# mattpan-peregrinus/Cosmology_GNN_Simulation

Measured on AMD Instinct MI355X. Metric: particle-edge updates/sec (E x MP-steps), higher is better.
Workload: dtype bf16; 1 GPU; 1000000 particles/GPU (1000000 in all, weak scaling) uniform periodic box, k=16, latent=128, hidden=128, 10 MP rounds, edge MLP bf16 (f32 accumulate, f32 latents/LayerNorm/residual), node path fp16x2, message_source=x_j; particles_per_gpu=1000000, edges_per_gpu=16000000, k=16, latent=128, mp_steps=10, parallelism=single GPU

## Files before the change

cosmology_gnn_simulation_amd/_lib.py:

```python
from __future__ import annotations

import ctypes as C
import os
from typing import Optional

import torch

_HERE = os.path.dirname(os.path.abspath(__file__))
LIB_PATH = os.path.join(_HERE, "libcgnn_hip.so")

MAX_HIDDEN_LAYERS = 6
F32, BF16, BF16_N16, F32X3, F32X3_N16, F16X2_N16, F16X2 = 0, 1, 2, 3, 4, 5, 6
N16_NODE = (F32X3_N16, F16X2_N16)
P_F32, P_BF16_S32, P_BF16_S16, P_F16_S32 = 0, 1, 2, 3
STREAM_FOLDED = 1
LDS_WEIGHT_BUDGET = 152 * 1024
PRECISIONS = {"fp32": F32, "f32": F32, "float32": F32, "bf16": BF16, "bfloat16": BF16, "bf16_n16": BF16_N16,
              "fp32x3": F32X3, "f32x3": F32X3, "fp32x3_n16": F32X3_N16, "fp16x2_n16": F16X2_N16,
              "fp16x2": F16X2, "f16x2": F16X2}
F32_EMULATED = (F32X3, F16X2)

EXPORTS = (
    "cgnn_version", "cgnn_arch", "cgnn_last_error", "cgnn_packed_linear_bytes", "cgnn_pack_linear",
    "cgnn_mlp_rows", "cgnn_project_nodes", "cgnn_edge_block", "cgnn_aggregate", "cgnn_node_block",
    "cgnn_knn_workspace_bytes", "cgnn_knn_periodic", "cgnn_knn_sorted_order", "cgnn_segment_colsum",
    "cgnn_gather_rows", "cgnn_scatter_rows", "cgnn_tiled_rows", "cgnn_relayout", "cgnn_window_features",
    "cgnn_mlp_backward", "cgnn_weight_grad", "cgnn_weight_grad_x3_workspace_bytes", "cgnn_weight_grad_x3",
    "cgnn_col_dot", "cgnn_col_dot2", "cgnn_col_dot_workspace_bytes", "cgnn_col_dot_ordered", "cgnn_weight_grad_workspace_bytes", "cgnn_weight_grad_ordered", "cgnn_csr_workspace_bytes", "cgnn_csr_build",
    "cgnn_aggregate_csr", "cgnn_aggregate_csr_add", "cgnn_edge_stream", "cgnn_edge_stream_image_bytes", "cgnn_edge_stream_image_build",
    "cgnn_edge_stream_run", "cgnn_edge_stream_w8_supported", "cgnn_edge_stream_image_build_w8", "cgnn_edge_stream_run_w8", "cgnn_aggregate_plan_bytes", "cgnn_aggregate_plan_build", "cgnn_aggregate_planned", "cgnn_aggregate_planned_rows",
    "cgnn_aggregate_planned_form", "cgnn_edge_mlp_backward", "cgnn_linear2_rows", "cgnn_halo_return_add", "cgnn_window_features_rows",
    "cgnn_rollout_integrate", "cgnn_frame_unpack", "cgnn_training_sample",
    "cgnn_balanced_planes_workspace_bytes", "cgnn_balanced_planes", "cgnn_tile_classify",
    "cgnn_knn_adaptive_workspace_bytes", "cgnn_knn_periodic_adaptive", "cgnn_knn_adaptive_sorted_order",
    "cgnn_history_features", "cgnn_rollout_advance", "cgnn_halo_select", "cgnn_halo_pack", "cgnn_migrate_pack",
    "cgnn_migrate_unpack", "cgnn_knn_periodic_mode", "cgnn_knn_periodic_adaptive_mode",
    "cgnn_training_sample_backward", "cgnn_rollout_integrate_backward", "cgnn_edge_attr_backward",
    "cgnn_edge_attr_backward_rows", "cgnn_rows_to_frames", "cgnn_frame_grad_rows", "cgnn_mlp_rows_project",
    "cgnn_knn_batched_workspace_bytes", "cgnn_knn_periodic_batched", "cgnn_knn_batched_sorted_order",
    "cgnn_pair_counts_workspace_bytes", "cgnn_pair_counts", "cgnn_frame_errors_workspace_bytes", "cgnn_frame_errors",
    "cgnn_mass_assign", "cgnn_power_bin_ids", "cgnn_power_bins_workspace_bytes", "cgnn_power_bins",
    "cgnn_fof_labels_workspace_bytes", "cgnn_fof_labels", "cgnn_fof_catalogue", "cgnn_mass_assign_backward",
    "cgnn_mass_assign_weighted", "cgnn_mass_assign_weighted_backward",
    "cgnn_halo_match_workspace_bytes", "cgnn_halo_match", "cgnn_fof_group_sums",
    "cgnn_halo_profiles_workspace_bytes", "cgnn_halo_profiles",
    "cgnn_redshift_positions", "cgnn_power_multipoles_workspace_bytes", "cgnn_power_multipoles",
    "cgnn_pair_counts_smu_workspace_bytes", "cgnn_pair_counts_smu",
    "cgnn_pair_velocity_sums_workspace_bytes", "cgnn_pair_velocity_sums",
)
PAIR_COUNTS_MAX_BINS = 256
PAIR_COUNTS_SMU_MAX_BINS = 4096
PAIR_COUNTS_SMU_MAX_AXIS = 128
PAIR_VELOCITY_MAX_BINS = 64
MASS_ASSIGN_Q = 8192
MASS_ASSIGN_MAX_MESH = 512
MASS_ASSIGN_MAX_PARTICLES = 1 << 24
WEIGHT_BITS = 20
WEIGHTED_MAX_PARTICLES = 1 << 23
WEIGHTED_MAX_CHANNELS = 4
POWER_MAX_BINS = 256
POWER_MULTIPOLE_SUMS = 12
FOF_MAX_BINS = 256
FOF_DISP_UNITS = 1 << 30
HALO_MATCH_COLS = 6
GROUP_SUMS_MAX_CHANNELS = 4
HALO_PROFILES_MAX_BINS = 32
HALO_PROFILES_MAX_CHANNELS = 4
KNN_BATCH_GROUP = 64
KNN_EDGE_ATTR_REFERENCE, KNN_EDGE_ATTR_IMAGE = 0, 1
ROLLOUT_ROW = 5
MIGRATE_BLOCK = 256
MIGRATE_MAX_WORLD = 64
ROWS, TILED32 = 0, 1


class Linear(C.Structure):
    _fields_ = [("w", C.c_void_p), ("b", C.c_void_p), ("in_dim", C.c_int32), ("out_dim", C.c_int32)]


class Mlp(C.Structure):
    _fields_ = [("precision", C.c_int32), ("num_hidden_layers", C.c_int32),
                ("layer", Linear * (MAX_HIDDEN_LAYERS + 1)),
                ("ln_gamma", C.c_void_p), ("ln_beta", C.c_void_p)]


class MlpBwdBuffers(C.Structure):
    _fields_ = [("h", C.c_void_p * MAX_HIDDEN_LAYERS), ("g_a", C.c_void_p * MAX_HIDDEN_LAYERS),
                ("g_o", C.c_void_p), ("zhat", C.c_void_p)]


class CgnnError(RuntimeError):
    pass


_lib: Optional[C.CDLL] = None


def load() -> C.CDLL:
    global _lib
    if _lib is not None:
        return _lib
    if not os.path.isfile(LIB_PATH):
        raise CgnnError(
            f"{LIB_PATH} not found. Build the gfx950 kernels first: "
            "`python -c 'import __graft_entry__ as g; g.build()'` or "
            "`make -C cosmology_gnn_simulation_amd/csrc -j8`. There is no CPU fallback.")
    lib = C.CDLL(LIB_PATH)
    vp, i32, i64, sz, f32 = C.c_void_p, C.c_int32, C.c_int64, C.c_size_t, C.c_float
    lib.cgnn_version.restype = C.c_int
    lib.cgnn_arch.restype = C.c_char_p
    lib.cgnn_last_error.restype = C.c_char_p
    lib.cgnn_packed_linear_bytes.restype = sz
    lib.cgnn_packed_linear_bytes.argtypes = [i32, i32, i32]
    lib.cgnn_pack_linear.argtypes = [vp, i32, i32, i32, i32, i32, vp, vp]
    lib.cgnn_mlp_rows.argtypes = [C.POINTER(Mlp), vp, i64, i32, vp, i32, i32, vp]
    lib.cgnn_mlp_rows_project.argtypes = [C.POINTER(Mlp), vp, vp, i64, i32, vp, i32, C.POINTER(Linear), C.POINTER(Linear),
                                          i32, vp, vp, i32, vp]
    lib.cgnn_tiled_rows.restype = i64
    lib.cgnn_tiled_rows.argtypes = [i64]
    lib.cgnn_relayout.argtypes = [vp, i32, vp, i32, i64, i32, vp]
    lib.cgnn_project_nodes.argtypes = [C.POINTER(Linear), C.POINTER(Linear), i32, vp, i64, vp, vp, i32, vp]
    lib.cgnn_edge_block.argtypes = [C.POINTER(Mlp), vp, vp, vp, vp, i64, vp, vp, vp, i32, i32, vp, vp, i32, vp]
    lib.cgnn_edge_stream.argtypes = [C.POINTER(Mlp), i32, vp, vp, i64, vp, vp, i64, vp, vp, i32, C.POINTER(Mlp), vp, i32, vp]
    lib.cgnn_edge_stream_image_bytes.restype = sz
    lib.cgnn_edge_stream_image_bytes.argtypes = [i32, i32, i32, i32]
    lib.cgnn_edge_stream_image_build.argtypes = [C.POINTER(Mlp), i32, C.POINTER(Mlp), i32, vp, sz, vp]
    lib.cgnn_edge_stream_run.argtypes = [vp, sz, i32, i32, i32, i32, vp, vp, i64, vp, vp, i64, vp, vp, vp, i32, vp]
    lib.cgnn_edge_stream_w8_supported.argtypes = [i32, i32, i32]
    lib.cgnn_edge_stream_image_build_w8.argtypes = [C.POINTER(Mlp), i32, C.POINTER(Mlp), i32, vp, sz, vp]
    lib.cgnn_edge_stream_run_w8.argtypes = [vp, sz, i32, i32, i32, i32, vp, vp, i64, vp, vp, i64, vp, vp, vp, i32, i32, i32, i32, i32, vp]
    lib.cgnn_aggregate.argtypes = [vp, i32, vp, vp, i64, i32, i64, i32, vp, vp]
    lib.cgnn_aggregate_plan_bytes.restype = sz
    lib.cgnn_aggregate_plan_bytes.argtypes = [i64, i32]
    lib.cgnn_aggregate_plan_build.argtypes = [vp, i64, i32, vp, vp]
    lib.cgnn_aggregate_planned.argtypes = [vp, vp, vp, i64, i32, i32, vp, vp]
    lib.cgnn_aggregate_planned_rows.argtypes = [vp, i64, vp, vp, i64, i32, i32, vp, vp]
    lib.cgnn_aggregate_planned_form.restype = i32
    lib.cgnn_aggregate_planned_form.argtypes = [i64, i64, i32, i32]
    lib.cgnn_node_block.argtypes = [C.POINTER(Mlp), C.POINTER(Linear), C.POINTER(Linear), vp, vp, i64, vp, i32, i32,
                                    C.POINTER(Linear), C.POINTER(Linear), i32, vp, vp, i32, vp]
    lib.cgnn_knn_workspace_bytes.restype = sz
    lib.cgnn_knn_workspace_bytes.argtypes = [i64, i32]
    lib.cgnn_knn_periodic.argtypes = [vp, i64, f32, i32, vp, i64, vp, vp, vp, sz, vp]
    lib.cgnn_knn_sorted_order.argtypes = [vp, i64, vp, vp]
    lib.cgnn_knn_adaptive_workspace_bytes.restype = sz
    lib.cgnn_knn_adaptive_workspace_bytes.argtypes = [i64, i32]
    lib.cgnn_knn_periodic_adaptive.argtypes = [vp, i64, f32, i32, vp, i64, vp, vp, vp, sz, vp]
    lib.cgnn_knn_adaptive_sorted_order.argtypes = [vp, i64, vp, vp]
    lib.cgnn_knn_periodic_mode.argtypes = lib.cgnn_knn_periodic.argtypes + [i32]
    lib.cgnn_knn_periodic_adaptive_mode.argtypes = lib.cgnn_knn_periodic_adaptive.argtypes + [i32]
    lib.cgnn_knn_batched_workspace_bytes.restype = sz
    lib.cgnn_knn_batched_workspace_bytes.argtypes = [C.POINTER(i64), i32, i32]
    lib.cgnn_knn_periodic_batched.argtypes = [vp, C.POINTER(i64), i32, f32, i32, vp, vp, vp, sz, vp, i32]
    lib.cgnn_knn_batched_sorted_order.argtypes = [vp, C.POINTER(i64), i32, vp, vp]
    lib.cgnn_pair_counts_workspace_bytes.restype = sz
    lib.cgnn_pair_counts_workspace_bytes.argtypes = [i64, i64, i32]
    lib.cgnn_pair_counts.argtypes = [vp, i64, vp, i64, f32, C.POINTER(f32), i32, vp, vp, sz, vp]
    lib.cgnn_pair_counts_smu_workspace_bytes.restype = sz
    lib.cgnn_pair_counts_smu_workspace_bytes.argtypes = [i64, i64, i32, i32]
    lib.cgnn_pair_counts_smu.argtypes = [vp, i64, vp, i64, f32, C.POINTER(f32), i32, C.POINTER(f32), i32, i32, vp, vp, sz,
                                         vp]
    lib.cgnn_pair_velocity_sums_workspace_bytes.restype = sz
    lib.cgnn_pair_velocity_sums_workspace_bytes.argtypes = [i64, i64, i32]
    lib.cgnn_pair_velocity_sums.argtypes = [vp, vp, i64, vp, vp, i64, f32, C.POINTER(f32), i32, vp, vp, vp, sz,
                                            vp]
    lib.cgnn_frame_errors_workspace_bytes.restype = sz
    lib.cgnn_frame_errors_workspace_bytes.argtypes = [i64, i64]
    lib.cgnn_frame_errors.argtypes = [vp, vp, vp, vp, i64, i64, f32, vp, vp, sz, vp]
    lib.cgnn_mass_assign.argtypes = [vp, i64, i64, f32, i32, i32, vp, vp]
    lib.cgnn_mass_assign_backward.argtypes = [vp, vp, i64, i64, f32, i32, i32, C.c_double, vp, vp]
    lib.cgnn_mass_assign_weighted.argtypes = [vp, vp, i64, i64, i32, f32, i32, i32, vp, vp]
    lib.cgnn_mass_assign_weighted_backward.argtypes = [vp, vp, vp, i64, i64, i32, f32, i32, i32, C.c_double, C.c_double,
                                                       vp, vp, vp]
    lib.cgnn_fof_labels_workspace_bytes.restype = sz
    lib.cgnn_fof_labels_workspace_bytes.argtypes = [i64]
    lib.cgnn_fof_labels.argtypes = [vp, i64, f32, f32, vp, vp, sz, vp]
    lib.cgnn_fof_catalogue.argtypes = [vp, vp, i64, f32, vp, vp, C.POINTER(i32), i32, vp, vp]
    lib.cgnn_halo_match_workspace_bytes.restype = sz
    lib.cgnn_halo_match_workspace_bytes.argtypes = [i64]
    lib.cgnn_halo_match.argtypes = [vp, vp, vp, vp, i64, i32, i32, vp, vp, vp, vp, C.POINTER(i32), i32, vp, vp, sz,
                                    vp]
    lib.cgnn_fof_group_sums.argtypes = [vp, vp, i64, i32, vp, vp]
    lib.cgnn_halo_profiles_workspace_bytes.restype = sz
    lib.cgnn_halo_profiles_workspace_bytes.argtypes = [i64, i64]
    lib.cgnn_halo_profiles.argtypes = [vp, i64, vp, i64, f32, C.POINTER(f32), i32, vp, i32, vp, vp, vp, sz,
                                       vp]
    lib.cgnn_power_bin_ids.argtypes = [i32, C.POINTER(f32), i32, vp, vp]
    lib.cgnn_power_bins_workspace_bytes.restype = sz
    lib.cgnn_power_bins_workspace_bytes.argtypes = [i64, i32]
    lib.cgnn_power_bins.argtypes = [vp, vp, i64, i32, i32, vp, vp, i32, vp, vp, vp, sz, vp]
    lib.cgnn_redshift_positions.argtypes = [vp, vp, i64, i64, f32, i32, f32, vp, vp]
    lib.cgnn_power_multipoles_workspace_bytes.restype = sz
    lib.cgnn_power_multipoles_workspace_bytes.argtypes = [i64, i32]
    lib.cgnn_power_multipoles.argtypes = [vp, vp, vp, vp, i64, i32, i32, i32, vp, vp, i32, vp, vp, vp, sz, vp]
    lib.cgnn_segment_colsum.argtypes = [vp, vp, i64, i32, i32, vp, vp]
    lib.cgnn_window_features.argtypes = [vp, vp, vp, vp, i32, i64, f32, f32, f32, f32, f32, f32, vp, vp, vp]
    lib.cgnn_window_features_rows.argtypes = [vp, vp, i32, i64, vp, i64, f32, f32, f32, f32, f32, f32, vp, vp, vp]
    lib.cgnn_rollout_integrate.argtypes = [vp, vp, vp, i64, vp, vp, vp, i64, i64, vp, f32, f32, vp, vp]
    lib.cgnn_frame_unpack.argtypes = [vp, i64, i64, vp, vp, vp]
    lib.cgnn_training_sample.argtypes = [vp, vp, vp, vp, i32, i64, vp, i64, C.c_double, C.c_uint64, C.c_uint64, f32, f32,
                                         f32, f32, f32, f32, vp, vp, vp, vp, vp, vp, vp, vp]
    lib.cgnn_training_sample_backward.argtypes = [vp, vp, vp, vp, i32, i64, vp, i64, i32, f32, f32, f32, f32, vp, vp, vp,
                                                  vp]
    lib.cgnn_rollout_integrate_backward.argtypes = [vp, vp, i64, vp, f32, f32, vp, vp, vp, vp, vp, vp]
    lib.cgnn_edge_attr_backward.argtypes = [vp, vp, vp, i64, i32, vp, vp, vp, vp]
    lib.cgnn_edge_attr_backward_rows.argtypes = [vp, vp, vp, i64, i64, i32, vp, vp, vp, vp]
    lib.cgnn_rows_to_frames.argtypes = [vp, vp, vp, i32, i64, i64, vp, vp, vp]
    lib.cgnn_frame_grad_rows.argtypes = [vp, vp, i64, i64, vp, vp, vp]
    lib.cgnn_balanced_planes_workspace_bytes.restype = sz
    lib.cgnn_balanced_planes_workspace_bytes.argtypes = [i64, i32, i32, i32]
    lib.cgnn_balanced_planes.argtypes = [vp, i64, i32, i32, i32, vp, vp, vp, vp, vp, sz, vp]
    lib.cgnn_tile_classify.argtypes = [vp, i64, i32, i32, i32, vp, vp, vp, i32, C.POINTER(C.c_double),
                                       C.POINTER(C.c_double), C.c_double, C.c_double, vp, vp, vp, vp]
    dp = C.POINTER(C.c_double)
    lib.cgnn_history_features.argtypes = [vp, i32, i64, i64, i32, vp, i64, vp, f32, f32, f32, f32, f32, f32, vp, vp, vp]
    lib.cgnn_rollout_advance.argtypes = [vp, i32, i64, i64, i32, vp, vp, vp, vp, i64, vp, f32, f32, i32, i32, i32, i32, vp,
                                         vp, vp, vp, vp, vp, vp, vp]
    lib.cgnn_halo_select.argtypes = [vp, i64, i32, i32, dp, dp, C.c_double, C.c_double, vp, vp, vp, vp]
    lib.cgnn_halo_pack.argtypes = [vp, vp, i64, i32, vp, i64, vp, vp]
    lib.cgnn_migrate_pack.argtypes = [vp, i32, i64, i64, vp, vp, i32, i32, vp, vp, i64, vp, vp, i64, vp]
    lib.cgnn_migrate_unpack.argtypes = [vp, i64, i32, vp, i64, i64, vp, vp]
    lib.cgnn_gather_rows.argtypes = [vp, vp, i64, i32, vp, vp]
    lib.cgnn_scatter_rows.argtypes = [vp, vp, i64, i32, vp, vp]
    lib.cgnn_halo_return_add.argtypes = [vp, i64, vp, vp, vp, i64, i32, vp, i64, vp]
    lib.cgnn_mlp_backward.argtypes = [C.POINTER(Mlp), C.POINTER(Linear), C.POINTER(Mlp), C.POINTER(Linear), vp, i32, vp,
                                      i32, vp, i32, i64, C.POINTER(MlpBwdBuffers), vp, i32, vp, i32, vp]
    lib.cgnn_edge_mlp_backward.argtypes = [C.POINTER(Mlp), C.POINTER(Mlp), vp, vp, vp, vp, i64, vp, vp, vp,
                                           C.POINTER(MlpBwdBuffers), vp, vp, i32, vp]
    lib.cgnn_linear2_rows.argtypes = [C.POINTER(Linear), C.POINTER(Linear), i32, vp, vp, i64, vp, vp, vp, vp]
    lib.cgnn_weight_grad.argtypes = [vp, i32, i32, vp, i32, i32, i64, vp, i32, i32, vp, vp]
    lib.cgnn_csr_workspace_bytes.restype = sz
    lib.cgnn_csr_workspace_bytes.argtypes = [i64]
    lib.cgnn_csr_build.argtypes = [vp, vp, i64, i64, vp, vp, vp, sz, vp]
    lib.cgnn_aggregate_csr.argtypes = [vp, vp, vp, i64, i32, vp, vp]
    lib.cgnn_aggregate_csr_add.argtypes = [vp, vp, vp, i64, i32, vp, vp, vp, vp]
    lib.cgnn_weight_grad_x3_workspace_bytes.argtypes = []
    lib.cgnn_weight_grad_x3_workspace_bytes.restype = C.c_size_t
    lib.cgnn_weight_grad_x3.argtypes = [vp, i32, vp, i32, i64, vp, i32, i32, vp, vp, C.c_size_t, vp]
    lib.cgnn_col_dot.argtypes = [vp, i32, vp, i32, i64, i32, vp, vp]
    lib.cgnn_col_dot2.argtypes = [vp, i32, vp, i32, i64, i32, vp, vp, vp]
    lib.cgnn_col_dot_workspace_bytes.restype = sz
    lib.cgnn_weight_grad_workspace_bytes.restype = sz
    lib.cgnn_weight_grad_workspace_bytes.argtypes = [i64, i32, i32]
    lib.cgnn_weight_grad_ordered.argtypes = [vp, i32, i32, vp, i32, i32, i64, vp, i32, i32, vp, vp, sz, vp]
    lib.cgnn_col_dot_workspace_bytes.argtypes = [i64, i32]
    lib.cgnn_col_dot_ordered.argtypes = [vp, i32, vp, i32, i64, i32, vp, vp, vp, sz, vp]
    missing = [name for name in EXPORTS if not hasattr(lib, name)]
    if missing:
        raise CgnnError(f"{LIB_PATH} lacks {missing}: rebuild it (make -C cosmology_gnn_simulation_amd/csrc)")
    _lib = lib
    return lib


def check(rc: int, what: str) -> None:
    if rc != 0:
        msg = load().cgnn_last_error().decode("utf-8", "replace")
        raise CgnnError(f"{what} failed (status {rc}): {msg}")


def require_device(t: torch.Tensor, name: str) -> None:
    if not t.is_cuda:
        raise CgnnError(f"{name} must live on a HIP device (got {t.device}); this engine has no CPU path")


def stream_ptr(device: torch.device) -> int:
    return torch.cuda.current_stream(device).cuda_stream


def ptr(t: Optional[torch.Tensor]) -> Optional[int]:
    return None if t is None else t.data_ptr()


def f32c(t: torch.Tensor, name: str) -> torch.Tensor:
    require_device(t, name)
    if t.dtype != torch.float32:
        t = t.float()
    return t if t.is_contiguous() else t.contiguous()


def i32c(t: torch.Tensor, name: str) -> torch.Tensor:
    require_device(t, name)
    if t.dtype != torch.int32:
        t = t.to(torch.int32)
    return t if t.is_contiguous() else t.contiguous()
```

cosmology_gnn_simulation_amd/csrc/edge_stream32w.hip:

```cpp
#include <string.h>

#include <type_traits>

#include "s32.hpp"

namespace cgnn {

#define CGNN_W8_WAVES 8
#define CGNN_W8_BLOCK (CGNN_W8_WAVES * 64)
#define CGNN_W8_SLOTS 3
#define CGNN_IC(x) std::integral_constant<int, (x)> {}
#include "w8_dev.hpp"

template <int DT>
struct W8Geom {
    typedef S32Geom<DT> G;
    static constexpr int D = G::D, KS = G::KS;
    static constexpr unsigned STRIDE = G::STRIDE, VEC_OFF = G::VEC_OFF;
    static constexpr int PIECES = (int)(STRIDE / 1024u);
    static constexpr int NP = (PIECES + CGNN_W8_WAVES - 1) / CGNN_W8_WAVES;
    static constexpr unsigned LNBUF_OFF = CGNN_W8_SLOTS * STRIDE;
    static constexpr unsigned LNBUF_BYTES = 2u * D * 4u;
    static constexpr unsigned PDST_OFF = LNBUF_OFF + 2u * LNBUF_BYTES;
    static constexpr unsigned PDST_ROW = 256u + 16u;
    static constexpr unsigned PDST_BYTES = 4u * PDST_ROW;
    static constexpr unsigned PSST_OFF = PDST_OFF + CGNN_W8_WAVES * PDST_BYTES;
    static constexpr unsigned PSST_BYTES = 64u * (unsigned)D / 2u;
    static constexpr unsigned LDS = PSST_OFF + CGNN_W8_WAVES * PSST_BYTES;
    static_assert(LDS <= 160u * 1024u, "LDS budget");
};

template <class W, int LAG>
struct RingW {
    const char* image;
    int count;
    int wave, lane;
    int slot;
    int dma_chunk, dma_slot;
    CGNN_W8_STAMP_MEMBER
    __device__ __forceinline__ RingW(const char* img, int cnt, int w, int l)
        : image(img), count(cnt), wave(w), lane(l), slot(0), dma_chunk(0), dma_slot(0) {}
    __device__ __forceinline__ unsigned lds0() const { return (unsigned)(uintptr_t)(LdsWeightPtr)(cgnn_smem); }
    __device__ __forceinline__ unsigned base() const { return lds0() + (unsigned)slot * W::STRIDE; }
    __device__ __forceinline__ unsigned base_next() const {
        return lds0() + (unsigned)(slot + 1 == CGNN_W8_SLOTS ? 0 : slot + 1) * W::STRIDE;
    }
    __device__ __forceinline__ unsigned vec_addr() const { return base() + W::VEC_OFF; }
    __device__ __forceinline__ unsigned lnbuf(int which) const { return lds0() + W::LNBUF_OFF + (unsigned)which * W::LNBUF_BYTES; }
    __device__ __forceinline__ void piece(int i) {
        asm volatile("" ::: "memory");
#if defined(__HIP_DEVICE_COMPILE__)
        int idx = wave + CGNN_W8_WAVES * i;
        if (idx >= W::PIECES) idx -= CGNN_W8_WAVES;
        const unsigned off = (unsigned)idx * 1024u;
        char* dst = cgnn_smem + (unsigned)dma_slot * W::STRIDE + off;
        const __amdgpu_buffer_rsrc_t rsrc =
            __builtin_amdgcn_make_buffer_rsrc(const_cast<char*>(image), 0, (int)((unsigned)count * W::STRIDE), 0x00020000);
        __builtin_amdgcn_raw_ptr_buffer_load_lds(rsrc, (LdsVoidPtrG)dst, 16, (unsigned)lane * 16u,
                                                 (unsigned)dma_chunk * W::STRIDE + off, 0, 0);
#endif
        asm volatile("" ::: "memory");
    }
    __device__ __forceinline__ void dma_done() {
        dma_chunk = dma_chunk + 1 == count ? 0 : dma_chunk + 1;
        dma_slot = dma_slot + 1 == CGNN_W8_SLOTS ? 0 : dma_slot + 1;
    }
    __device__ __forceinline__ void prime() {
        for (int c = 0; c < CGNN_W8_SLOTS - 1 - LAG; ++c) {
            for (int i = 0; i < W::NP; ++i) piece(i);
            dma_done();
        }
        CGNN_S32_VMCNT(0);
        __builtin_amdgcn_s_barrier();
        asm volatile("" ::: "memory");
    }
    template <int EXTRA, int K0 = 17>
    __device__ __forceinline__ void interval_end() {
        CGNN_W8_STAMP(K0);
        if constexpr (w8dev::SLEEP > 0) __builtin_amdgcn_s_sleep(w8dev::SLEEP);
        vm_wait_const<(LAG ? 0 : (CGNN_W8_CARRY ? EXTRA : W::NP + EXTRA))>();
        asm volatile("s_waitcnt lgkmcnt(0)" ::: "memory");
        CGNN_W8_STAMP(K0 + 1);
        __builtin_amdgcn_s_barrier();
        asm volatile("" ::: "memory");
        CGNN_W8_STAMP(K0 + 2);
    }
    __device__ __forceinline__ void advance() { slot = slot + 1 == CGNN_W8_SLOTS ? 0 : slot + 1; }
    __device__ __forceinline__ void idle_interval() {
        for (int i = 0; i < W::NP; ++i) piece(i);
        dma_done();
        interval_end<0>();
    }
};

template <int N>
__device__ __forceinline__ void lds_wait2(u32x4& a, u32x4& b) {
    asm volatile("s_waitcnt lgkmcnt(%2)" : "+v"(a), "+v"(b) : "n"(N));
}

struct FragBuf {
    static constexpr int PD = CGNN_W8_PD, NBUF = PD + 1;
    u32x4 b[NBUF][CGNN_W8_GS];
};
template <int M>
struct WBlockGeom {
    static constexpr int GS = CGNN_W8_GS, NG = M / GS;
    static_assert(M % GS == 0 && (GS == 4 || GS == 2), "groups of four or two fragments");
    static constexpr int rot_after(int rot) { return (rot + NG) % FragBuf::NBUF; }
};
template <int M, int ROT>
__device__ __forceinline__ void wblock_request(FragBuf& fb, unsigned addr) {
    constexpr int GS = WBlockGeom<M>::GS, NG = WBlockGeom<M>::NG, PD = FragBuf::PD, NBUF = FragBuf::NBUF;
    const unsigned a = addr + (unsigned)(threadIdx.x & 63) * 16u;
    static_for_each([&](auto pc) __attribute__((always_inline)) {
        constexpr int p = decltype(pc)::value;
        if constexpr (p < NG) {
            static_for_each([&](auto jc) __attribute__((always_inline)) {
                constexpr int j = decltype(jc)::value;
                fb.b[(ROT + p) % NBUF][j] = lds_read_b128<(p * GS + j) * 1024>(a);
            }, std::make_integer_sequence<int, GS>{});
        }
    }, std::make_integer_sequence<int, PD>{});
}
template <int NROW, int KS, int ROT, bool CIN, bool COUT, class Fill>
__device__ __forceinline__ void wblockw(f32x16 (&acc)[NROW], const bf16x8 (&in)[KS], FragBuf& fb, unsigned addr, unsigned addr_next,
                                        const Fill& fill) {
    constexpr int M = NROW * KS, GS = WBlockGeom<M>::GS, NG = WBlockGeom<M>::NG, PD = FragBuf::PD, NBUF = FragBuf::NBUF;
    static_assert(!COUT || NG >= PD, "a block that requests the next one's fragments is at least PD groups long");
    const unsigned a = addr + (unsigned)(threadIdx.x & 63) * 16u;
    const unsigned an = addr_next + (unsigned)(threadIdx.x & 63) * 16u;
    (void)an;
    if constexpr (!CIN) wblock_request<M, ROT>(fb, addr);
    static_for_each([&](auto gc) __attribute__((always_inline)) {
        constexpr int g = decltype(gc)::value;
        constexpr int newer = COUT ? (PD - 1) * GS : ((g + PD - 1 < NG ? g + PD - 1 : NG - 1) - g) * GS;
        constexpr int bi = (ROT + g) % NBUF;
        if constexpr (GS == 4)
            lds_wait4<newer>(fb.b[bi][0], fb.b[bi][1], fb.b[bi][2], fb.b[bi][3]);
        else
            lds_wait2<newer>(fb.b[bi][0], fb.b[bi][1]);
        static_for_each([&](auto jc) __attribute__((always_inline)) {
            constexpr int j = decltype(jc)::value, m = g * GS + j, o = m / KS, ks = m % KS;
            acc[o] = __builtin_amdgcn_mfma_f32_32x32x16_bf16(__builtin_bit_cast(bf16x8, fb.b[bi][j]), in[ks], acc[o], 0, 0, 0);
            if constexpr (g + PD < NG)
                fb.b[(ROT + g + PD) % NBUF][j] = lds_read_b128<((g + PD) * GS + j) * 1024>(a);
            else if constexpr (COUT)
                fb.b[(ROT + g + PD) % NBUF][j] = lds_read_b128<((g + PD - NG) * GS + j) * 1024>(an);
            fill.template run<m>();
            __builtin_amdgcn_sched_barrier(0);
        }, std::make_integer_sequence<int, GS>{});
    }, std::make_integer_sequence<int, NG>{});
}

template <bool RELU, int DT, int T, int S>
__device__ __forceinline__ void packw_slice(bf16x8 (&out)[2 * DT], const f32x16 (&acc)[DT]) {
    u32x4 v;
    v[0] = pack_bf16(acc[T][8 * S + 0], acc[T][8 * S + 1]);
    v[1] = pack_bf16(acc[T][8 * S + 2], acc[T][8 * S + 3]);
    v[2] = pack_bf16(acc[T][8 * S + 4], acc[T][8 * S + 5]);
    v[3] = pack_bf16(acc[T][8 * S + 6], acc[T][8 * S + 7]);
    const bf16x8 b = __builtin_bit_cast(bf16x8, v);
    out[2 * T + S] = RELU ? relu_bf16(b) : b;
}

template <int DT, int T0, int T1>
__device__ __forceinline__ void bias_rowsw(f32x16 (&acc)[DT], unsigned vec_addr, int h) {
    if constexpr (w8dev::ABL_BIAS) return;
    const LdsVecPtr b = (LdsVecPtr)(uintptr_t)vec_addr;
#pragma unroll
    for (int t = T0; t < T1; ++t)
#pragma unroll
        for (int g = 0; g < 4; ++g) {
            const f32x4 v = *(LdsVec4Ptr)(b + 32 * t + 8 * g + 4 * h);
#pragma unroll
            for (int c = 0; c < 4; ++c) acc[t][4 * g + c] = v[c];
        }
}

struct LnStats {
    float rstd, nmr;
};
struct LnSums {
    float s[4], q[4];
};
__device__ __forceinline__ void ln_sums_clear(LnSums& a) {
#pragma unroll
    for (int i = 0; i < 4; ++i) a.s[i] = a.q[i] = 0.f;
}
template <bool ZM, int DT, int T, int S>
__device__ __forceinline__ void ln_sums_add(LnSums& a, const f32x16 (&acc)[DT]) {
#pragma unroll
    for (int i = 8 * S; i < 8 * S + 8; i += 4) {
#pragma unroll
        for (int c = 0; c < 4; ++c) {
            if constexpr (!ZM) a.s[c] += acc[T][i + c];
            a.q[c] = __builtin_fmaf(acc[T][i + c], acc[T][i + c], a.q[c]);
        }
    }
}
template <bool ZM, int DT>
__device__ __forceinline__ LnStats ln_stats_finish(const LnSums& a) {
    constexpr int D = 32 * DT;
    const float ex2 = half_swap_sum((a.q[0] + a.q[1]) + (a.q[2] + a.q[3])) * (1.0f / D);
    LnStats st;
    if constexpr (ZM) {
        st.rstd = __builtin_amdgcn_rsqf(ex2 + 1e-5f);
        st.nmr = 0.f;
    } else {
        const float mean = half_swap_sum((a.s[0] + a.s[1]) + (a.s[2] + a.s[3])) * (1.0f / D);
        st.rstd = __builtin_amdgcn_rsqf(__builtin_fmaxf(__builtin_fmaf(-mean, mean, ex2), 0.f) + 1e-5f);
        st.nmr = -mean * st.rstd;
    }
    return st;
}
template <bool RES, bool BETA, bool ZM, int DT, int K0, int K1>
__device__ __forceinline__ void ln_affine_w(const f32x16 (&acc)[DT], f32x16 (&ev)[DT], bf16x8 (&in)[2 * DT], unsigned lnv, int h,
                                            LnStats st) {
    if constexpr (K1 > K0) {
        constexpr int D = 32 * DT;
        const LdsVecPtr gp = (LdsVecPtr)(uintptr_t)lnv + 4 * h;
        f32x4 gm[2][2], bt[2][2];
#pragma unroll
        for (int gg = 0; gg < 2; ++gg) {
            gm[K0 & 1][gg] = *(LdsVec4Ptr)(gp + 32 * (K0 >> 1) + 8 * (2 * (K0 & 1) + gg));
            if constexpr (BETA) bt[K0 & 1][gg] = *(LdsVec4Ptr)(gp + D + 32 * (K0 >> 1) + 8 * (2 * (K0 & 1) + gg));
        }
        __builtin_amdgcn_sched_barrier(0);
        static_for_each([&](auto kc) __attribute__((always_inline)) {
            constexpr int k = decltype(kc)::value + K0, t = k >> 1, s = k & 1, cur = k & 1, nxt = cur ^ 1;
            if constexpr (k + 1 < K1) {
                constexpr int t1 = (k + 1) >> 1, s1 = (k + 1) & 1;
#pragma unroll
                for (int gg = 0; gg < 2; ++gg) {
                    gm[nxt][gg] = *(LdsVec4Ptr)(gp + 32 * t1 + 8 * (2 * s1 + gg));
                    if constexpr (BETA) bt[nxt][gg] = *(LdsVec4Ptr)(gp + D + 32 * t1 + 8 * (2 * s1 + gg));
                }
            }
            if constexpr (w8dev::ABL_LN) {
                packw_slice<false, DT, t, s>(in, acc);
#pragma unroll
                for (int i = 0; i < 8; ++i) ev[t][8 * s + i] += acc[t][8 * s + i];
            } else {
                float nrm[8], bs[8];
#pragma unroll
                for (int i = 0; i < 8; ++i) nrm[i] = ZM ? acc[t][8 * s + i] * st.rstd : __builtin_fmaf(acc[t][8 * s + i], st.rstd, st.nmr);
                __builtin_amdgcn_sched_barrier(0);
                if constexpr (BETA) {
#pragma unroll
                    for (int i = 0; i < 8; ++i) bs[i] = RES ? bt[cur][i >> 2][i & 3] + ev[t][8 * s + i] : bt[cur][i >> 2][i & 3];
                    __builtin_amdgcn_sched_barrier(0);
                } else {
                    static_assert(BETA || RES, "a pass without beta adds into the residual");
#pragma unroll
                    for (int i = 0; i < 8; ++i) bs[i] = ev[t][8 * s + i];
                }
#pragma unroll
                for (int i = 0; i < 8; ++i) ev[t][8 * s + i] = __builtin_fmaf(nrm[i], gm[cur][i >> 2][i & 3], bs[i]);
                __builtin_amdgcn_sched_barrier(0);
                u32x4 v;
#pragma unroll
                for (int x = 0; x < 4; ++x) v[x] = pack_bf16(ev[t][8 * s + 2 * x], ev[t][8 * s + 2 * x + 1]);
                in[2 * t + s] = __builtin_bit_cast(bf16x8, v);
            }
            __builtin_amdgcn_sched_barrier(0);
        }, std::make_integer_sequence<int, K1 - K0>{});
    }
}

template <int DT, int T0, int T1>
__device__ __forceinline__ void selp_rows(f32x16 (&acc)[DT], const bf16x8 (&ps)[2 * DT], const bf16x8 (&pd)[2 * DT], bf16x8 sel0,
                                          bf16x8 sel1) {
    if constexpr (w8dev::ABL_SEL) return;
    static_for_each([&](auto tc) __attribute__((always_inline)) {
        constexpr int t = decltype(tc)::value + T0;
        f32x16 c = {0.f, 0.f, 0.f, 0.f, 0.f, 0.f, 0.f, 0.f, 0.f, 0.f, 0.f, 0.f, 0.f, 0.f, 0.f, 0.f};
        c = __builtin_amdgcn_mfma_f32_32x32x16_bf16(sel0, ps[2 * t], c, 0, 0, 0);
        c = __builtin_amdgcn_mfma_f32_32x32x16_bf16(sel1, ps[2 * t + 1], c, 0, 0, 0);
        c = __builtin_amdgcn_mfma_f32_32x32x16_bf16(sel0, pd[2 * t], c, 0, 0, 0);
        c = __builtin_amdgcn_mfma_f32_32x32x16_bf16(sel1, pd[2 * t + 1], c, 0, 0, 0);
        acc[t] = c;
    }, std::make_integer_sequence<int, T1 - T0>{});
}

__device__ __forceinline__ float mix_add_lo(unsigned a, unsigned b) {
    float r;
    asm("v_fma_mix_f32 %0, %1, 1.0, %2 op_sel:[0,0,0] op_sel_hi:[1,0,1]" : "=v"(r) : "v"(a), "v"(b));
    return r;
}
__device__ __forceinline__ float mix_add_hi(unsigned a, unsigned b) {
    float r;
    asm("v_fma_mix_f32 %0, %1, 1.0, %2 op_sel:[1,0,1] op_sel_hi:[1,0,1]" : "=v"(r) : "v"(a), "v"(b));
    return r;
}
template <int DT, int T, int S>
__device__ __forceinline__ void addp_half(f32x16 (&acc)[DT], const bf16x8 (&ps)[2 * DT], const bf16x8 (&pd)[2 * DT]) {
    const u32x4 a = __builtin_bit_cast(u32x4, ps[2 * T + S]), b = __builtin_bit_cast(u32x4, pd[2 * T + S]);
#pragma unroll
    for (int x = 0; x < 4; ++x) {
        acc[T][8 * S + 2 * x] = mix_add_lo(a[x], b[x]);
        acc[T][8 * S + 2 * x + 1] = mix_add_hi(a[x], b[x]);
    }
}
template <int DT, int T0, int T1>
__device__ __forceinline__ void addp_rows(f32x16 (&acc)[DT], const bf16x8 (&ps)[2 * DT], const bf16x8 (&pd)[2 * DT]) {
    static_for_each([&](auto tc) __attribute__((always_inline)) {
        constexpr int t = decltype(tc)::value + T0;
#pragma unroll
        for (int s = 0; s < 2; ++s) {
            const u32x4 a = __builtin_bit_cast(u32x4, ps[2 * t + s]), b = __builtin_bit_cast(u32x4, pd[2 * t + s]);
#pragma unroll
            for (int x = 0; x < 4; ++x) {
                acc[t][8 * s + 2 * x] = mix_add_lo(a[x], b[x]);
                acc[t][8 * s + 2 * x + 1] = mix_add_hi(a[x], b[x]);
            }
        }
    }, std::make_integer_sequence<int, T1 - T0>{});
}

template <int DT, int NH, bool ENC, int LAG, bool PF16, bool FOLD>
__global__ __launch_bounds__(CGNN_W8_BLOCK, 2) void edge_stream32w_kernel(
    S32Args a, const __bf16* __restrict__ ps_all, const __bf16* __restrict__ pd_all, int64_t round_stride,
    const int32_t* __restrict__ src, const int32_t* __restrict__ dst, int64_t num_edges, const float* e_in, float* e_out,
    const float* __restrict__ attr, int ld_attr, int seg_k) {
    typedef W8Geom<DT> W;
    static_assert(DT == 4, "the sender-row staging is laid out for latent 128 (four lanes per 64-byte half line)");
    constexpr int D = W::D, KS = W::KS, NP = W::NP;
    const int lane = threadIdx.x & 63, r = lane & 31, h = lane >> 5;
    const int wave = __builtin_amdgcn_readfirstlane(threadIdx.x >> 6);
    const bool lagging = LAG != 0 && wave >= CGNN_W8_WAVES / 2;
    const int L = a.rounds;
    const int steps_per_tile = (ENC ? NH + 1 : 0) + L * (NH + 1);
    const int64_t tiles = (num_edges + 31) / 32;
    const TileRange tr = tile_range(tiles);
    const int64_t first0 = tr.first - wave;
    const int iters = __builtin_amdgcn_readfirstlane(
        first0 < tr.end ? (int)((tr.end - first0 + tr.stride - 1) / tr.stride) : 0);
    if (iters == 0) return;
    RingW<W, LAG> ring(a.image, steps_per_tile, wave, lane);
    CGNN_W8_STAMP_BEGIN(ring)
    ring.prime();
    if (lagging) ring.idle_interval();
    const bf16x8 sel0 = p32_selector(lane, 0), sel1 = p32_selector(lane, 1);

    f32x16 ev[DT], acc[DT];
    FragBuf fb;
    constexpr bool CARRY = CGNN_W8_CARRY && LAG == 0;
    auto rot_at = [](bool enc_first, int l) constexpr -> int {
        int r = 0;
        if (l >= 1) r = enc_first ? WBlockGeom<DT * 2>::rot_after(0) : WBlockGeom<DT * KS>::rot_after(0);
        for (int i = 1; i < l; ++i) r = WBlockGeom<DT * KS>::rot_after(r);
        return r;
    };
    (void)rot_at;
    bf16x8 inb[2][2 * DT];
    bf16x8 ps[2 * DT], pd[2 * DT];
    int lnpar = 0;
    LnStats lnst = {0.f, 0.f};
    constexpr int KA = CGNN_W8_LN_EARLY < 2 * DT ? CGNN_W8_LN_EARLY : 2 * DT;
    int64_t tile = tr.first < tr.end ? tr.first : tr.end - 1;
    bool valid = tr.first < tr.end;

    const unsigned pdst = ring.lds0() + W::PDST_OFF + (unsigned)wave * W::PDST_BYTES;
    const int kk = seg_k < 32 ? seg_k : 32;
    auto load_pd_chunk = [&](const __bf16* table, unsigned off) __attribute__((always_inline)) -> u32x4 {
#if defined(__HIP_DEVICE_COMPILE__)
        const __amdgpu_buffer_rsrc_t rsrc = __builtin_amdgcn_make_buffer_rsrc(const_cast<__bf16*>(table), 0, 0x7fffffff, 0x00020000);
        return __builtin_amdgcn_raw_buffer_load_b128(rsrc, (int)off, 0, 0);
#else
        return u32x4{0u, 0u, 0u, 0u};
#endif
    };
    auto park_pd = [&](u32x4 chunk) __attribute__((always_inline)) {
        *(__attribute__((address_space(3))) u32x4*)(uintptr_t)(pdst + (unsigned)(lane >> 4) * W::PDST_ROW + (unsigned)(lane & 15) * 16u) = chunk;
    };
    const unsigned pd_read = pdst + (unsigned)(r / kk) * W::PDST_ROW + (PF16 ? 4u : 8u) * (unsigned)h * 16u;
    auto pd_piece = [](int i) constexpr -> unsigned { return PF16 ? (unsigned)(((i >> 2) * 8 + (i & 3)) * 16) : (unsigned)(16 * i); };
    auto read_pd = [&]() __attribute__((always_inline)) {
#pragma unroll
        for (int i = 0; i < 2 * DT; ++i)
            pd[i] = __builtin_bit_cast(bf16x8, *(const __attribute__((address_space(3))) u32x4*)(uintptr_t)(pd_read + pd_piece(i)));
    };
    auto read_pd_row = [&](auto tc) __attribute__((always_inline)) {
        constexpr int t = decltype(tc)::value;
#pragma unroll
        for (int i = 2 * t; i < 2 * t + 2; ++i)
            pd[i] = __builtin_bit_cast(bf16x8, *(const __attribute__((address_space(3))) u32x4*)(uintptr_t)(pd_read + pd_piece(i)));
    };
    u32x4 pdchunk = {0u, 0u, 0u, 0u};

    const unsigned psst = ring.lds0() + W::PSST_OFF + (unsigned)wave * W::PSST_BYTES;
    const unsigned ps_cq = (unsigned)((lane & 3) ^ ((lane >> 4) & 3)) * 16u;
    const unsigned ps_read = psst + (unsigned)(r + 32 * h) * 64u + (unsigned)((r >> 2) & 3) * 16u;
    unsigned so_lo = 0, so_hi = 0;
    auto stage_ps = [&](auto sub_c, auto i_c, const __bf16* table) __attribute__((always_inline)) {
        constexpr int SUB = decltype(sub_c)::value, i = decltype(i_c)::value;
        (void)SUB, (void)i, (void)ps_cq;
        asm volatile("" ::: "memory");
#if defined(__HIP_DEVICE_COMPILE__)
        const __amdgpu_buffer_rsrc_t rsrc = __builtin_amdgcn_make_buffer_rsrc(const_cast<__bf16*>(table), 0, 0x7fffffff, 0x00020000);
        char* dstp = cgnn_smem + W::PSST_OFF + (unsigned)wave * W::PSST_BYTES + (unsigned)i * 1024u;
        __builtin_amdgcn_raw_ptr_buffer_load_lds(rsrc, (LdsVoidPtrG)dstp, 16, ((i & 1) ? so_hi : so_lo) + ps_cq,
                                                 PF16 ? (i >> 1) * 64 + SUB * 128 : (i >> 1) * D + SUB * 64, 0, 0);
#endif
        asm volatile("" ::: "memory");
    };
    auto read_ps = [&](auto sub_c) __attribute__((always_inline)) {
        constexpr int SUB = decltype(sub_c)::value;
#pragma unroll
        for (int c = 0; c < 4; ++c)
            ps[4 * SUB + c] = __builtin_bit_cast(
                bf16x8, *(const __attribute__((address_space(3))) u32x4*)(uintptr_t)(ps_read ^ ((unsigned)c << 4)));
    };
    auto pieces_at = [&](auto qc, auto mc) __attribute__((always_inline)) {
        constexpr int q = decltype(qc)::value, M = decltype(mc)::value;
        constexpr int P0 = CGNN_W8_PIECE_SLOT + NP <= M ? CGNN_W8_PIECE_SLOT : M - NP;
        if constexpr (q >= P0 && q < P0 + NP) ring.piece(q - P0);
    };

    struct TileIn {
        int src_lo, src_hi, dst_row;
        f32x4 q;
    };
    auto load_tile_in = [&](int64_t T, TileIn& ti) __attribute__((always_inline)) {
        const int64_t e = T * 32 + r;
        const int64_t ce = e < num_edges ? e : num_edges - 1;
        const int64_t e_lo = T * 32 + (lane >> 2), e_hi = e_lo + 16;
        ti.src_lo = src[e_lo < num_edges ? e_lo : num_edges - 1];
        ti.src_hi = src[e_hi < num_edges ? e_hi : num_edges - 1];
        const int groups = 32 / kk;
        const int j = (lane >> 4) < groups ? (lane >> 4) : groups - 1;
        const int64_t eg = T * 32 + (int64_t)j * kk;
        ti.dst_row = dst[eg < num_edges ? eg : num_edges - 1];
        if (ENC) ti.q = *reinterpret_cast<const f32x4*>(attr + ce * ld_attr);
    };
    TileIn nxt;
    load_tile_in(tile, nxt);

    for (int it = 0; it < iters; ++it) {
        const unsigned dchunk = (unsigned)nxt.dst_row * (unsigned)D * 2u + (unsigned)(lane & 15) * 16u;
        const int64_t tn = tile + tr.stride;
        const int64_t tile_next = tn < tr.end ? tn : tile;
        {
            so_lo = (unsigned)nxt.src_lo * (unsigned)D * 2u;
            so_hi = (unsigned)nxt.src_hi * (unsigned)D * 2u;
            const f32x4 q_now = nxt.q;
            load_tile_in(tile_next, nxt);
            if (ENC) {
                const int fin = a.enc_in_dim;
                float v[8];
#pragma unroll
                for (int jj = 0; jj < 8; ++jj) v[jj] = (jj < 4 && h == 0 && jj < fin) ? q_now[jj] : 0.f;
                u32x4 w;
                w[0] = pack_bf16(v[0], v[1]);
                w[1] = pack_bf16(v[2], v[3]);
                w[2] = pack_bf16(v[4], v[5]);
                w[3] = pack_bf16(v[6], v[7]);
                inb[0][0] = __builtin_bit_cast(bf16x8, w);
                const u32x4 z = {0u, 0u, 0u, 0u};
                inb[0][1] = __builtin_bit_cast(bf16x8, z);
            } else {
                load_tile<DT>(ev, e_in + tile * (32 * D), lane);
#pragma unroll
                for (int t = 0; t < DT; ++t)
#pragma unroll
                    for (int s = 0; s < 2; ++s) {
                        u32x4 w;
#pragma unroll
                        for (int x = 0; x < 4; ++x) w[x] = pack_bf16(ev[t][8 * s + 2 * x], ev[t][8 * s + 2 * x + 1]);
                        inb[0][2 * t + s] = __builtin_bit_cast(bf16x8, w);
                    }
                park_pd(load_pd_chunk(pd_all, dchunk));
                static_for_each([&](auto ic) __attribute__((always_inline)) { stage_ps(CGNN_IC(0), ic, ps_all); },
                                std::make_integer_sequence<int, 4>{});
                CGNN_S32_VMCNT(0);
                read_ps(CGNN_IC(0));
                asm volatile("s_waitcnt lgkmcnt(0)" ::: "memory");
                static_for_each([&](auto ic) __attribute__((always_inline)) { stage_ps(CGNN_IC(1), ic, ps_all); },
                                std::make_integer_sequence<int, 4>{});
                CGNN_S32_VMCNT(0);
                read_ps(CGNN_IC(1));
                read_pd();
            }
        }

        auto step_first = [&](auto enc_tag, auto pend_tag, int rr) __attribute__((always_inline)) {
            constexpr bool IS_ENC = decltype(enc_tag)::value;
            constexpr int PEND = decltype(pend_tag)::value;
            constexpr int KS0 = IS_ENC ? 2 : KS;
            constexpr bool INBLK = PF16 && CGNN_W8_PF16_INBLK && NH <= 2 && !IS_ENC && PEND != 0;
            CGNN_W8_STAMP(8);
            if constexpr (PEND != 0) {
                if constexpr (!IS_ENC) {
                    if constexpr (LAG == 0) CGNN_S32_VMCNT(0);
                    park_pd(pdchunk);
                    read_ps(CGNN_IC(0));
                    asm volatile("s_waitcnt lgkmcnt(0)" ::: "memory");
                    const __bf16* tps = ps_all + (int64_t)rr * round_stride;
                    static_for_each([&](auto ic) __attribute__((always_inline)) { stage_ps(CGNN_IC(1), ic, tps); },
                                    std::make_integer_sequence<int, 4>{});
                }
                ln_affine_w<PEND == 2, !(FOLD && PEND == 2), FOLD, DT, KA, 2 * DT>(acc, ev, inb[0], ring.lnbuf(lnpar ^ 1), h, lnst);
                if constexpr (!IS_ENC) {
                    if constexpr (INBLK) read_pd_row(CGNN_IC(0)); else read_pd();
                }
            }
            const unsigned base = ring.base();
            CGNN_W8_STAMP(9);
            constexpr bool REQ = CARRY && !IS_ENC && CGNN_W8_REQ_EARLY;
            if constexpr (REQ) wblock_request<DT * KS0, 0>(fb, base);
            if constexpr (IS_ENC) {
                bias_rowsw<DT, 0, DT>(acc, ring.vec_addr() + (unsigned)D * 4u, h);
            } else if constexpr (PEND != 0) {
                if constexpr (INBLK) {
                    addp_rows<DT, 0, 1>(acc, ps, pd);
                } else if constexpr (PF16) {
                    addp_rows<DT, 0, DT / 2>(acc, ps, pd);
                    CGNN_S32_VMCNT(0);
                    read_ps(CGNN_IC(1));
                    addp_rows<DT, DT / 2, DT>(acc, ps, pd);
                } else {
                    selp_rows<DT, 0, DT / 2>(acc, ps, pd, sel0, sel1);
                    CGNN_S32_VMCNT(0);
                    read_ps(CGNN_IC(1));
                    selp_rows<DT, DT / 2, DT>(acc, ps, pd, sel0, sel1);
                }
            } else {
                if constexpr (PF16) addp_rows<DT, 0, DT>(acc, ps, pd);
                else selp_rows<DT, 0, DT>(acc, ps, pd, sel0, sel1);
            }
            CGNN_W8_STAMP(10);
            const bf16x8 (&in0)[KS0] = reinterpret_cast<const bf16x8(&)[KS0]>(inb[0][0]);
            wblockw<DT, KS0, 0, REQ, CARRY>(acc, in0, fb, base, ring.base_next(), make_fill([&](auto qc) __attribute__((always_inline)) {
                constexpr int q = decltype(qc)::value, t = q / KS0 - 1, w = q % KS0;
                pieces_at(qc, CGNN_IC(DT * KS0));
                if constexpr (INBLK && t + 2 < DT) {
                    constexpr int tn = t + 2 < DT ? t + 2 : 0;
                    if constexpr (w == 0) {
                        if constexpr (tn == DT / 2) {
                            CGNN_S32_VMCNT(0);
                            read_ps(CGNN_IC(1));
                        }
                        read_pd_row(CGNN_IC(tn));
                    }
                    if constexpr (w == CGNN_W8_ADDP0) addp_half<DT, tn, 0>(acc, ps, pd);
                    if constexpr (w == CGNN_W8_ADDP1) addp_half<DT, tn, 1>(acc, ps, pd);
                }
                if constexpr (t >= 0 && w == (KS0 > 4 ? CGNN_W8_PK0 : (KS0 > 2 ? 1 : KS0 - 1))) packw_slice<true, DT, (t < 0 ? 0 : t), 0>(inb[1], acc);
                if constexpr (t >= 0 && w == (KS0 > 4 ? CGNN_W8_PK1 : KS0 - 1)) {
                    packw_slice<true, DT, (t < 0 ? 0 : t), 1>(inb[1], acc);
                    bias_rowsw<DT, (t < 0 ? 0 : t), (t < 0 ? 0 : t) + 1>(acc, ring.vec_addr(), h);
                }
            }));
            packw_slice<true, DT, DT - 1, 0>(inb[1], acc);
            packw_slice<true, DT, DT - 1, 1>(inb[1], acc);
            bias_rowsw<DT, DT - 1, DT>(acc, ring.vec_addr(), h);
            ring.dma_done();
            ring.template interval_end<0, 11>();
            ring.advance();
        };
        auto step_hidden = [&](auto enc_tag, auto lc) __attribute__((always_inline)) {
            constexpr int l = decltype(lc)::value;
            constexpr bool IS_ENC = decltype(enc_tag)::value;
            CGNN_W8_STAMP(14);
            wblockw<DT, KS, rot_at(IS_ENC, l), CARRY, CARRY>(acc, inb[l & 1], fb, ring.base(), ring.base_next(), make_fill([&](auto qc) __attribute__((always_inline)) {
                constexpr int q = decltype(qc)::value, t = q / KS - 1, w = q % KS;
                pieces_at(qc, CGNN_IC(DT * KS));
                if constexpr (t >= 0 && w == (KS > 4 ? CGNN_W8_PK0 : (KS > 2 ? 1 : KS - 1))) packw_slice<true, DT, (t < 0 ? 0 : t), 0>(inb[(l + 1) & 1], acc);
                if constexpr (t >= 0 && w == (KS > 4 ? CGNN_W8_PK1 : KS - 1)) {
                    packw_slice<true, DT, (t < 0 ? 0 : t), 1>(inb[(l + 1) & 1], acc);
                    bias_rowsw<DT, (t < 0 ? 0 : t), (t < 0 ? 0 : t) + 1>(acc, ring.vec_addr(), h);
                }
            }));
            packw_slice<true, DT, DT - 1, 0>(inb[(l + 1) & 1], acc);
            packw_slice<true, DT, DT - 1, 1>(inb[(l + 1) & 1], acc);
            bias_rowsw<DT, DT - 1, DT>(acc, ring.vec_addr(), h);
            ring.dma_done();
            ring.template interval_end<0, 15>();
            ring.advance();
        };
        auto step_last = [&](auto enc_tag, auto p_tag, auto res_tag, const __bf16* nps, const __bf16* npd) __attribute__((always_inline)) {
            constexpr bool WITH_P = decltype(p_tag)::value, RES = decltype(res_tag)::value, IS_ENC = decltype(enc_tag)::value;
            CGNN_W8_STAMP(0);
            CGNN_W8_STAMP(1);
            LnSums sums;
            ln_sums_clear(sums);
            wblockw<DT, KS, rot_at(IS_ENC, NH), CARRY, false>(acc, inb[NH & 1], fb, ring.base(), 0u, make_fill([&](auto qc) __attribute__((always_inline)) {
                constexpr int q = decltype(qc)::value, t = q / KS - 1, w = q % KS;
                pieces_at(qc, CGNN_IC(DT * KS));
                constexpr int PQ = CGNN_W8_PIECE_SLOT == 0 ? NP : 0;
                if constexpr (WITH_P && q >= PQ && q < PQ + 4) stage_ps(CGNN_IC(0), CGNN_IC(q - PQ), nps);
                if constexpr (WITH_P && q == PQ + 4) pdchunk = load_pd_chunk(npd, dchunk);
                if constexpr (t >= 0 && w == (KS > 4 ? CGNN_W8_SM0 : (KS > 2 ? 2 : KS - 1))) ln_sums_add<FOLD, DT, (t < 0 ? 0 : t), 0>(sums, acc);
                if constexpr (t >= 0 && w == (KS > 4 ? CGNN_W8_SM1 : KS - 1)) ln_sums_add<FOLD, DT, (t < 0 ? 0 : t), 1>(sums, acc);
            }));
            CGNN_W8_STAMP(2);
            ln_sums_add<FOLD, DT, DT - 1, 0>(sums, acc);
            ln_sums_add<FOLD, DT, DT - 1, 1>(sums, acc);
            lnst = ln_stats_finish<FOLD, DT>(sums);
            ln_affine_w<RES, !(FOLD && RES && WITH_P), FOLD, DT, 0, KA>(acc, ev, inb[0], ring.vec_addr() + (unsigned)D * 4u, h, lnst);
            if (wave < CGNN_W8_WAVES / 2) {
                const int idx = wave * 64 + lane;
                if (idx < 2 * D) {
                    const LdsVecPtr sp = (LdsVecPtr)(uintptr_t)(ring.vec_addr() + (unsigned)D * 4u);
                    const float v = sp[idx];
                    ((__attribute__((address_space(3))) float*)(uintptr_t)ring.lnbuf(lnpar))[idx] = v;
                }
            }
            lnpar ^= 1;
            ring.dma_done();
            ring.template interval_end<(WITH_P && (!CARRY || CGNN_W8_PIECE_SLOT == 0) ? 5 : 0), 3>();
            ring.advance();
        };
        auto hidden_steps = [&](auto enc_tag) __attribute__((always_inline)) {
            static_for_each([&](auto lc) __attribute__((always_inline)) {
                step_hidden(enc_tag, std::integral_constant<int, decltype(lc)::value + 1>{});
            }, std::make_integer_sequence<int, NH - 1>{});
        };
        constexpr std::true_type ENC_PASS{};
        constexpr std::false_type ROUND_PASS{};

        if (ENC) {
            step_first(ENC_PASS, CGNN_IC(0), 0);
            hidden_steps(ENC_PASS);
            step_last(ENC_PASS, std::true_type{}, std::false_type{}, ps_all, pd_all);
            step_first(ROUND_PASS, CGNN_IC(1), 0);
            hidden_steps(ROUND_PASS);
        } else {
            step_first(ROUND_PASS, CGNN_IC(0), 0);
            hidden_steps(ROUND_PASS);
        }
        for (int rr = 1; rr < L; ++rr) {
            step_last(ROUND_PASS, std::true_type{}, std::true_type{}, ps_all + (int64_t)rr * round_stride, pd_all + (int64_t)rr * round_stride);
            step_first(ROUND_PASS, CGNN_IC(2), rr);
            hidden_steps(ROUND_PASS);
        }
        step_last(ROUND_PASS, std::false_type{}, std::true_type{}, ps_all, pd_all);
        ln_affine_w<true, true, FOLD, DT, KA, 2 * DT>(acc, ev, inb[0], ring.lnbuf(lnpar ^ 1), h, lnst);

        if (valid) {
            float* const tb = e_out + tile * (32 * D);
#pragma unroll
            for (int t = 0; t < DT; ++t)
#pragma unroll
                for (int g = 0; g < 4; ++g) {
                    const f32x4 v = {ev[t][4 * g], ev[t][4 * g + 1], ev[t][4 * g + 2], ev[t][4 * g + 3]};
                    __builtin_nontemporal_store(v, reinterpret_cast<f32x4*>(tb + ((4 * t + g) * 64 + lane) * 4));
                }
        }
        if (tn < tr.end) {
            tile = tn;
        } else {
            valid = false;
        }
    }
    if (LAG != 0 && !lagging) ring.idle_interval();
    CGNN_W8_STAMP_END(wave, lane)
    CGNN_S32_VMCNT(0);
    __builtin_amdgcn_s_barrier();
}

template <int DT, int NH, int LAG, bool PF16, bool FOLD>
static int launch_w8(const S32Args& a, const __bf16* ps, const __bf16* pd, int64_t round_stride, const int32_t* src,
                     const int32_t* dst, int64_t num_edges, const float* e_in, float* e_out, const float* attr, int ld_attr,
                     int seg_k, hipStream_t st) {
    typedef W8Geom<DT> W;
    const bool enc = a.enc_in_dim > 0;
    auto kern = enc ? edge_stream32w_kernel<DT, NH, true, LAG, PF16, FOLD> : edge_stream32w_kernel<DT, NH, false, LAG, PF16, FOLD>;
    if (W::LDS > 48 * 1024) {
        int rc = ensure_dynamic_lds(reinterpret_cast<const void*>(kern), W::LDS, "hipFuncSetAttribute(edge_stream32w)");
        if (rc != CGNN_OK) return rc;
    }
    const int64_t tiles = (num_edges + 31) / 32;
    const int grid = grid_for_tiles(tiles, 1, CGNN_W8_WAVES);
    kern<<<grid, CGNN_W8_BLOCK, W::LDS, st>>>(a, ps, pd, round_stride, src, dst, num_edges, e_in, e_out, attr, ld_attr, seg_k);
    CGNN_W8_STAMP_REPORT(st, num_edges, grid, a.rounds + (enc ? 1 : 0), LAG)
    return check_hip(hipGetLastError(), "cgnn_edge_stream_run_w8 launch");
}

}

using namespace cgnn;

extern "C" int cgnn_edge_stream_image_build_w8(const cgnn_mlp* rounds, int32_t num_rounds, const cgnn_mlp* encoder,
                                               int32_t latent, void* image, size_t image_bytes, void* stream) {
    int rc = cgnn_edge_stream_image_build(rounds, num_rounds, encoder, latent, image, image_bytes, stream);
    if (rc != CGNN_OK) return rc;
    const size_t stride = s32_stride(latent);
    const int nh = rounds[0].num_hidden_layers;
    const int count = (num_rounds + (encoder ? 1 : 0)) * (nh + 1);
    hipStream_t st = (hipStream_t)stream;
    const size_t vbytes = (size_t)latent * 4, voff = (size_t)latent * latent * 2;
    char* img = (char*)image;
    rc = check_hip(hipMemcpyAsync(img + voff + vbytes, img + voff, vbytes, hipMemcpyDeviceToDevice, st), "hipMemcpyAsync(own bias)");
    for (int c = 0; c + 1 < count && rc == CGNN_OK; ++c)
        rc = check_hip(hipMemcpyAsync(img + (size_t)c * stride + voff, img + (size_t)(c + 1) * stride + voff, vbytes,
                                      hipMemcpyDeviceToDevice, st), "hipMemcpyAsync(bias, one chunk early)");
    if (rc == CGNN_OK) rc = check_hip(hipMemsetAsync(img + (size_t)(count - 1) * stride + voff, 0, vbytes, st), "hipMemsetAsync(last bias)");
    return rc;
}

extern "C" int cgnn_edge_stream_w8_supported(int32_t latent, int32_t num_hidden_layers, int32_t fixed_k) {
    const bool k_ok = fixed_k >= 8 && (fixed_k <= 32 ? 32 % fixed_k == 0 : fixed_k % 32 == 0);
    return (latent == 128 && num_hidden_layers >= 1 && num_hidden_layers <= 3 && k_ok) ? 1 : 0;
}

extern "C" int cgnn_edge_stream_run_w8(const void* image, size_t image_bytes, int32_t latent, int32_t num_hidden_layers,
                                       int32_t num_rounds, int32_t enc_in_dim, const void* ps_all, const void* pd_all,
                                       int64_t round_stride, const int32_t* src, const int32_t* dst, int64_t num_edges,
                                       const float* e_in, float* e_out, const float* edge_attr, int32_t ld_attr, int32_t lag,
                                       int32_t fixed_k, int32_t p_format, int32_t flags, void* stream) {
    if (!image || !ps_all || !pd_all || !src || !dst || !e_out || num_edges < 0 || num_rounds < 1 || num_hidden_layers < 1 ||
        round_stride < 0 || (enc_in_dim > 0 ? (!edge_attr || ld_attr < enc_in_dim) : !e_in) || lag < 0 || lag > 1 || fixed_k < 0) {
        set_error("cgnn_edge_stream_run_w8: invalid argument");
        return CGNN_ERR_INVALID_ARG;
    }
    if (p_format != CGNN_P_BF16_S32 && p_format != CGNN_P_F16_S32) {
        set_error("cgnn_edge_stream_run_w8: ps_all / pd_all must be CGNN_P_F16_S32 or CGNN_P_BF16_S32 tables (got p_format %d)",
                  p_format);
        return CGNN_ERR_INVALID_ARG;
    }
    if ((flags & ~CGNN_STREAM_FOLDED) != 0 || ((flags & CGNN_STREAM_FOLDED) && p_format != CGNN_P_F16_S32)) {
        set_error("cgnn_edge_stream_run_w8: flags = %d (known: CGNN_STREAM_FOLDED, with CGNN_P_F16_S32 tables only)", flags);
        return CGNN_ERR_INVALID_ARG;
    }
    if (p_format == CGNN_P_F16_S32 && lag != 0) {
        set_error("cgnn_edge_stream_run_w8: fp16 tables (CGNN_P_F16_S32) run with lag = 0 (lag = 1 is kept for bf16 tables)");
        return CGNN_ERR_UNSUPPORTED;
    }
    if (enc_in_dim > 4 || (enc_in_dim > 0 && ((ld_attr & 3) != 0 || ((uintptr_t)edge_attr & 15) != 0))) {
        set_error("cgnn_edge_stream_run_w8: the in-launch encoder reads an edge's features with one aligned 16-byte load: at most "
                  "4 features (got %d), ld_attr a multiple of 4 (got %d), edge_attr 16-byte aligned; other layouts: "
                  "cgnn_edge_stream_run", enc_in_dim, ld_attr);
        return CGNN_ERR_UNSUPPORTED;
    }
    if (!cgnn_edge_stream_w8_supported(latent, num_hidden_layers, fixed_k) || num_edges % fixed_k != 0) {
        set_error("cgnn_edge_stream_run_w8: no kernel for latent=%d, %d hidden layers, fixed_k=%d on %lld edges (built for latent "
                  "128, 1..3 hidden layers of the same width and receiver-sorted edge lists of fixed in-degree 8, 16, 32, 64, ...; "
                  "other shapes: cgnn_edge_stream_run)", latent, num_hidden_layers, fixed_k, (long long)num_edges);
        return CGNN_ERR_UNSUPPORTED;
    }
    const size_t need = cgnn_edge_stream_image_bytes(latent, num_hidden_layers, num_rounds, enc_in_dim > 0);
    if (image_bytes < need) {
        set_error("cgnn_edge_stream_run_w8: image has %zu bytes, this model needs %zu", image_bytes, need);
        return CGNN_ERR_INVALID_ARG;
    }
    if (num_edges == 0) return CGNN_OK;
    S32Args a;
    a.image = (const char*)image;
    a.rounds = num_rounds;
    a.nh = num_hidden_layers;
    a.enc_in_dim = enc_in_dim > 0 ? enc_in_dim : 0;
    hipStream_t st = (hipStream_t)stream;
#define CGNN_W8_GO(NHx, LAGx, PFx, FOLDx)                                                                                    \
    return launch_w8<4, NHx, LAGx, PFx, FOLDx>(a, (const __bf16*)ps_all, (const __bf16*)pd_all, round_stride, src, dst, num_edges, \
                                               e_in, e_out, edge_attr, ld_attr, fixed_k, st)
    if (flags & CGNN_STREAM_FOLDED) {
        switch (num_hidden_layers) {
            case 1: CGNN_W8_GO(1, 0, true, true);
            case 2: CGNN_W8_GO(2, 0, true, true);
            default: CGNN_W8_GO(3, 0, true, true);
        }
    }
    if (p_format == CGNN_P_F16_S32) {
        switch (num_hidden_layers) {
            case 1: CGNN_W8_GO(1, 0, true, false);
            case 2: CGNN_W8_GO(2, 0, true, false);
            default: CGNN_W8_GO(3, 0, true, false);
        }
    }
    if (lag) {
        switch (num_hidden_layers) {
            case 1: CGNN_W8_GO(1, 1, false, false);
            case 2: CGNN_W8_GO(2, 1, false, false);
            default: CGNN_W8_GO(3, 1, false, false);
        }
    }
    switch (num_hidden_layers) {
        case 1: CGNN_W8_GO(1, 0, false, false);
        case 2: CGNN_W8_GO(2, 0, false, false);
        default: CGNN_W8_GO(3, 0, false, false);
    }
#undef CGNN_W8_GO
}
```

cosmology_gnn_simulation_amd/csrc/w8_dev.hpp:

```cpp
#pragma once

#ifndef CGNN_W8_GS
#define CGNN_W8_GS 2
#endif
#ifndef CGNN_W8_PD
#define CGNN_W8_PD 2
#endif
#ifndef CGNN_W8_LN_EARLY
#define CGNN_W8_LN_EARLY 0
#endif
#ifndef CGNN_W8_PK0
#define CGNN_W8_PK0 2
#define CGNN_W8_PK1 4
#endif
#ifndef CGNN_W8_SM0
#define CGNN_W8_SM0 4
#define CGNN_W8_SM1 6
#endif
#ifndef CGNN_W8_PIECE_SLOT
#define CGNN_W8_PIECE_SLOT 16
#endif
#ifndef CGNN_W8_CARRY
#define CGNN_W8_CARRY 1
#endif
#ifndef CGNN_W8_REQ_EARLY
#define CGNN_W8_REQ_EARLY 1
#endif
#ifndef CGNN_W8_PF16_INBLK
#define CGNN_W8_PF16_INBLK 1
#endif
#ifndef CGNN_W8_ADDP0
#define CGNN_W8_ADDP0 5
#define CGNN_W8_ADDP1 6
#endif

namespace w8dev {
#ifdef CGNN_W8_ABL_LN
constexpr bool ABL_LN = true;
#else
constexpr bool ABL_LN = false;
#endif
#ifdef CGNN_W8_ABL_SEL
constexpr bool ABL_SEL = true;
#else
constexpr bool ABL_SEL = false;
#endif
#ifdef CGNN_W8_ABL_BIAS
constexpr bool ABL_BIAS = true;
#else
constexpr bool ABL_BIAS = false;
#endif
#ifdef CGNN_W8_SLEEP
constexpr int SLEEP = CGNN_W8_SLEEP;
#else
constexpr int SLEEP = 0;
#endif
}

#ifdef CGNN_W8_STAMPS
#include <stdio.h>
__device__ unsigned long long cgnn_w8_stamps[8 * 32];
struct W8Timer {
    unsigned long long sum[20], prev;
};
#define CGNN_W8_STAMP_MEMBER W8Timer tm;
#define CGNN_W8_STAMP(k)                                                                 \
    {                                                                                    \
        unsigned long long t_;                                                           \
        __builtin_amdgcn_sched_barrier(0);                                               \
        asm volatile("s_memtime %0\n\ts_waitcnt lgkmcnt(0)" : "=s"(t_)::"memory");       \
        __builtin_amdgcn_sched_barrier(0);                                               \
        tm.sum[k] += t_ - tm.prev;                                                       \
        tm.prev = t_;                                                                    \
    }
#define CGNN_W8_STAMP_BEGIN(ring)                                                            \
    auto& tm = ring.tm;                                                                      \
    for (int k = 0; k < 20; ++k) tm.sum[k] = 0;                                              \
    asm volatile("s_memtime %0\n\ts_waitcnt lgkmcnt(0)" : "=s"(tm.prev)::"memory");
#define CGNN_W8_STAMP_END(wave, lane)  \
    if (blockIdx.x == 8 && lane == 0)  \
        for (int k = 0; k < 20; ++k) cgnn_w8_stamps[wave * 32 + k] = tm.sum[k];
#define CGNN_W8_STAMP_REPORT(st, num_edges, grid, passes_per_tile, lag)                                                           \
    {                                                                                                                             \
        static int printed = 0;                                                                                                   \
        (void)hipStreamSynchronize(st);                                                                                           \
        if (printed++ == 2) {                                                                                                     \
            static unsigned long long hs[8 * 32];                                                                                 \
            (void)hipMemcpyFromSymbol(hs, HIP_SYMBOL(cgnn_w8_stamps), sizeof(hs));                                                \
            const char* names[20] = {"(gap)", "last: bias, P requests", "last: MFMAs", "last: LayerNorm part, copy",              \
                                     "last: vmcnt wait", "last: barrier", "", "", "(gap; tile ends)", "first: LayerNorm rest, Pd", \
                                     "first: P sums", "first: L0 + pack", "first: vmcnt wait", "first: barrier", "(gap)",          \
                                     "hidden: bias, MFMAs, pack", "hidden: vmcnt wait", "hidden: barrier / idle interval",         \
                                     "idle: vmcnt", "idle: barrier"};                                                              \
            const double passes = (double)(((num_edges) + 31) / 32) / ((grid) * 8.0) * (passes_per_tile);                          \
            printf("lag %d: cycles per pass and wave, by phase (sums over the wave's whole run / %.0f passes)\n", lag, passes);    \
            double tot[8] = {0};                                                                                                  \
            for (int k = 0; k < 20; ++k) {                                                                                        \
                bool any = false;                                                                                                 \
                for (int w = 0; w < 8; ++w) any |= hs[w * 32 + k] != 0;                                                           \
                if (!any) continue;                                                                                               \
                printf("  %2d %-28s", k, names[k]);                                                                               \
                for (int w = 0; w < 8; ++w) {                                                                                     \
                    printf(" %7.0f", hs[w * 32 + k] / passes);                                                                    \
                    tot[w] += hs[w * 32 + k] / passes;                                                                            \
                }                                                                                                                 \
                printf("\n");                                                                                                     \
            }                                                                                                                     \
            printf("     %-28s", "total");                                                                                        \
            for (int w = 0; w < 8; ++w) printf(" %7.0f", tot[w]);                                                                 \
            printf("\n");                                                                                                         \
        }                                                                                                                         \
    }
#else
#define CGNN_W8_STAMP_MEMBER
#define CGNN_W8_STAMP(k)
#define CGNN_W8_STAMP_BEGIN(ring)
#define CGNN_W8_STAMP_END(wave, lane)
#define CGNN_W8_STAMP_REPORT(st, num_edges, grid, passes_per_tile, lag)
#endif
```

cosmology_gnn_simulation_amd/ops.py:

```python
from __future__ import annotations

import ctypes as C
import math
import weakref
from typing import List, Optional, Sequence, Tuple

import torch

from . import _lib
from ._lib import BF16, BF16_N16, F32, CgnnError, Linear, Mlp, check, f32c, i32c, ptr, require_device, stream_ptr


_timer = None


class OpTimer:

    def __init__(self):
        self.records = {}

    def __enter__(self):
        global _timer
        _timer = self
        return self
# ... 58 lines not shown
        out_dim, ld = w.shape
        ncols = ld - col0 if ncols is None else ncols
        self.precision = _prec(precision)
        self.in_dim, self.out_dim = int(ncols), int(out_dim)
        nbytes = lib.cgnn_packed_linear_bytes(out_dim, ncols, self.precision)
        self.packed = torch.empty(nbytes, dtype=torch.uint8, device=w.device)
        with _timed("pack_linear", w.device):
            check(lib.cgnn_pack_linear(w.data_ptr(), out_dim, ld, col0, ncols, self.precision, self.packed.data_ptr(),
                                       stream_ptr(w.device)), "cgnn_pack_linear")
        self.bias = None if bias is None else f32c(bias.detach(), "bias").clone()

    def struct(self) -> Linear:
        return Linear(self.packed.data_ptr(), ptr(self.bias), self.in_dim, self.out_dim)


class PackedMLP:

    def __init__(self, linears: Sequence[Tuple[torch.Tensor, Optional[torch.Tensor]]],
                 layer_norm: Optional[Tuple[torch.Tensor, torch.Tensor]], precision,
                 first_layer_cols: Optional[Tuple[int, int]] = None):
        nh = len(linears) - 1
        if nh < 1 or nh > _lib.MAX_HIDDEN_LAYERS:
            raise CgnnError(f"mlp_num_hidden_layers={nh} outside [1, {_lib.MAX_HIDDEN_LAYERS}]")
        self.precision = _prec(precision)
        self.layers: List[PackedLinear] = []
        for i, (w, b) in enumerate(linears):
            if i == 0 and first_layer_cols is not None:
                self.layers.append(PackedLinear(w, b, self.precision, first_layer_cols[0], first_layer_cols[1]))
            else:
                self.layers.append(PackedLinear(w, b, self.precision))
        self.gamma = self.beta = None
        if layer_norm is not None:
            self.gamma = f32c(layer_norm[0].detach(), "ln weight").clone()
            self.beta = f32c(layer_norm[1].detach(), "ln bias").clone()
        self.num_hidden_layers = nh
        self.in_dim = self.layers[0].in_dim
        self.hidden = self.layers[0].out_dim
        self.out_dim = self.layers[-1].out_dim
        m = Mlp()
        m.precision = self.precision
        m.num_hidden_layers = nh
        for i, L in enumerate(self.layers):
            m.layer[i] = L.struct()
        m.ln_gamma = ptr(self.gamma)
        m.ln_beta = ptr(self.beta)
        self._struct = m

    def struct(self) -> Mlp:
        return self._struct

    def lds_bytes(self) -> int:
        pad16 = lambda n: (n * 4 + 15) // 16 * 16
        return sum(L.packed.numel() for L in self.layers) + sum(pad16(L.out_dim) for L in self.layers) + \
            2 * pad16(self.out_dim)


class TiledRows:

    def __init__(self, n: int, width: int, device, buf: Optional[torch.Tensor] = None):
        if width % 32:
            raise CgnnError(f"TILED32 needs a width that is a multiple of 32 (got {width})")
        self.n, self.width = int(n), int(width)
        rows = ((self.n + 31) // 32) * 32
        self.buf = buf if buf is not None else torch.empty((rows, width), dtype=torch.float32, device=device)
        if self.buf.shape != (rows, width) or not self.buf.is_contiguous():
            raise CgnnError("TiledRows: buffer has the wrong shape")

    @property
    def device(self):
        return self.buf.device

    def empty_like(self) -> "TiledRows":
        return TiledRows(self.n, self.width, self.buf.device)

    def to_rows(self) -> torch.Tensor:
        return relayout(self)

    @staticmethod
    def from_rows(x: torch.Tensor) -> "TiledRows":
        return relayout(x)


def relayout(x, out: Optional[torch.Tensor] = None):
    lib = _lib.load()
    if isinstance(x, TiledRows):
        if out is None:
            out = torch.empty((x.n, x.width), dtype=torch.float32, device=x.device)
        elif out.dtype != torch.float32 or not out.is_contiguous() or out.dim() != 2 or out.shape[1] != x.width or \
                out.shape[0] < x.n or out.device != x.device:
            raise CgnnError("relayout: out must be contiguous float32 [>= n, width] on the tiles' device")
        if x.n:
            with _timed("relayout", x.device):
                check(lib.cgnn_relayout(x.buf.data_ptr(), _lib.TILED32, out.data_ptr(), _lib.ROWS, x.n, x.width,
                                        stream_ptr(x.device)), "cgnn_relayout")
        return out
    x = f32c(x, "x")
    t = TiledRows(x.shape[0], x.shape[1], x.device)
    if t.n:
        with _timed("relayout", x.device):
            check(lib.cgnn_relayout(x.data_ptr(), _lib.ROWS, t.buf.data_ptr(), _lib.TILED32, t.n, t.width,
                                    stream_ptr(x.device)), "cgnn_relayout")
    return t


def mlp_rows(mlp: PackedMLP, x: torch.Tensor, out=None, tiled: bool = False, next_projection=None,
             index: Optional[torch.Tensor] = None):
    if not (mlp.precision == _lib.F16X2_N16 and torch.is_tensor(x) and x.is_cuda and x.dtype == torch.float32 and
            x.dim() == 2 and x.stride(1) == 1 and x.stride(0) >= x.shape[1]):
        x = f32c(x, "x")
    if x.dim() != 2 or x.shape[1] != mlp.in_dim:
        raise CgnnError(f"mlp_rows: input is {tuple(x.shape)}, the MLP expects [n, {mlp.in_dim}]")
    n = x.shape[0] if index is None else int(index.numel())
    if tiled or isinstance(out, TiledRows):
        y = out if out is not None else TiledRows(n, mlp.out_dim, x.device)
        yb, layout = y.buf, _lib.TILED32
    else:
        y = out if out is not None else torch.empty((n, mlp.out_dim), dtype=torch.float32, device=x.device)
        yb, layout = y, _lib.ROWS
    if next_projection is None and index is None:
        with _timed("mlp_rows", x.device):
            check(_lib.load().cgnn_mlp_rows(C.byref(mlp.struct()), x.data_ptr(), n, x.stride(0), yb.data_ptr(),
                                            yb.stride(0), layout, stream_ptr(x.device)), "cgnn_mlp_rows")
        return y
    if mlp.precision != _lib.F16X2_N16 or layout != _lib.ROWS:
        raise CgnnError("mlp_rows: next_projection / index need an 'fp16x2_n16' pack and row-major output")
    if index is not None:
        index = i32c(index, "index")
        if y.shape[0] < n or (mlp.gamma is None and x.shape[0] < n):
            raise CgnnError("mlp_rows: index is longer than the rows it addresses")
    if next_projection is not None:
        ws, wd, ps, pd, p_format = next_projection
        s1, s2 = ws.struct(), wd.struct()
        pdt = p_format_dtype(p_format)
        for t in (ps, pd):
            require_device(t, "projection table")
            if t.dtype != pdt or not t.is_contiguous() or t.shape != (n, ws.out_dim):
                raise CgnnError("mlp_rows: projection tables have the wrong dtype/shape")
        proj = (C.byref(s1), C.byref(s2), ws.precision, ps.data_ptr(), pd.data_ptr(), p_format)
    else:
        ps = pd = None
        proj = (None, None, 0, None, None, 0)
    _same_device(x, index, y, ps, pd)
    with _timed("mlp_rows", x.device):
        check(_lib.load().cgnn_mlp_rows_project(C.byref(mlp.struct()), x.data_ptr(), ptr(index), n, x.stride(0),
                                                yb.data_ptr(), yb.stride(0), *proj, stream_ptr(x.device)),
              "cgnn_mlp_rows_project")
    return y


def p_table_format(edge_mlp_precision) -> int:
    return {F32: _lib.P_F32, BF16: _lib.P_BF16_S32, BF16_N16: _lib.P_BF16_S16,
            _lib.F16X2_N16: _lib.P_F32, _lib.F16X2: _lib.P_F32}[_prec(edge_mlp_precision)]


def p_format_dtype(p_format: int) -> torch.dtype:
    return {_lib.P_F32: torch.float32, _lib.P_F16_S32: torch.float16}.get(p_format, torch.bfloat16)


def p_table_dtype(edge_mlp_precision) -> torch.dtype:
    return torch.float32 if _prec(edge_mlp_precision) in (F32, _lib.F16X2_N16, _lib.F16X2) else torch.bfloat16


def project_nodes(ws: Optional[PackedLinear], wd: Optional[PackedLinear], x: torch.Tensor,
                  ps: Optional[torch.Tensor] = None, pd: Optional[torch.Tensor] = None,
                  p_format: Optional[int] = None):
    x = f32c(x, "x")
    n = x.shape[0]
    ref = ws if ws is not None else wd
    if p_format is None:
        p_format = p_table_format(ref.precision)
    pdt = p_format_dtype(p_format)
    if ws is not None and ps is None:
        ps = torch.empty((n, ws.out_dim), dtype=pdt, device=x.device)
    if wd is not None and pd is None:
        pd = torch.empty((n, wd.out_dim), dtype=pdt, device=x.device)
    for t in (ps, pd):
        if t is not None and (t.dtype != pdt or not t.is_contiguous()):
            raise CgnnError(f"project_nodes: tables must be contiguous {pdt} for this precision")
    s1 = ws.struct() if ws is not None else None
    s2 = wd.struct() if wd is not None else None
    with _timed("project_nodes", x.device):
        check(_lib.load().cgnn_project_nodes(C.byref(s1) if s1 is not None else None,
                                         C.byref(s2) if s2 is not None else None, ref.precision, x.data_ptr(), n,
                                         ptr(ps) if ws is not None else None, ptr(pd) if wd is not None else None,
                                         p_format, stream_ptr(x.device)), "cgnn_project_nodes")
    return ps, pd


def edge_block(mlp: PackedMLP, ps: torch.Tensor, pd: torch.Tensor, src: torch.Tensor, dst: torch.Tensor,
               e_in: TiledRows, e_out: Optional[TiledRows] = None, e_upd: Optional[TiledRows] = None,
               residual: bool = True, agg_out: Optional[torch.Tensor] = None, x_gather: Optional[torch.Tensor] = None,
               seg_k: int = 0) -> TiledRows:
    if not isinstance(e_in, TiledRows):
        raise CgnnError("edge_block: edge latents must be TiledRows (use ops.relayout / TiledRows.from_rows)")
    src, dst = i32c(src, "src"), i32c(dst, "dst")
    ne, latent = e_in.n, e_in.width
    if e_out is None:
        e_out = e_in.empty_like()
    for t, name in ((ps, "ps"), (pd, "pd")):
        require_device(t, name)
        if not t.is_contiguous() or t.dtype != p_table_dtype(mlp.precision):
            raise CgnnError(f"edge_block: {name} must be a contiguous project_nodes table of the MLP's precision")
    for t in (e_out, e_upd):
        if t is not None and (t.n != ne or t.width != latent):
            raise CgnnError("edge_block: e_out / e_upd do not match the edge latents")
    if src.numel() != ne or dst.numel() != ne:
        raise CgnnError("edge_block: src/dst length does not match the edge latents")
    if agg_out is not None:
        if x_gather is not None:
            x_gather = f32c(x_gather, "x_gather")
            if x_gather.shape[1] != latent:
                raise CgnnError("edge_block: x_gather width must equal the latent size")
        if agg_out.dtype != torch.float32 or not agg_out.is_contiguous() or agg_out.shape[1] != latent:
            raise CgnnError("edge_block: agg_out must be contiguous float32 [receivers, latent]")
    _same_device(ps, pd, src, dst, e_in.buf, e_out.buf, x_gather, agg_out)
    with _timed("edge_block", e_in.device):
        check(_lib.load().cgnn_edge_block(C.byref(mlp.struct()), ps.data_ptr(), pd.data_ptr(), src.data_ptr(),
                                          dst.data_ptr(), ne, e_in.buf.data_ptr(), e_out.buf.data_ptr(),
                                          None if e_upd is None else e_upd.buf.data_ptr(),
                                          1 if residual else 0, latent, ptr(x_gather), ptr(agg_out), seg_k,
                                          stream_ptr(e_in.device)), "cgnn_edge_block")
    return e_out


def edge_stream(mlps: Sequence[PackedMLP], ps_all: torch.Tensor, pd_all: torch.Tensor, src: torch.Tensor,
                dst: torch.Tensor, e_in: Optional[TiledRows], e_out: Optional[TiledRows] = None,
                encoder: Optional[PackedMLP] = None, edge_attr: Optional[torch.Tensor] = None) -> TiledRows:
    src, dst = i32c(src, "src"), i32c(dst, "dst")
    rounds = len(mlps)
    ne = src.numel()
    if encoder is not None:
        if edge_attr is None:
            raise CgnnError("edge_stream: the encoder needs edge_attr")
        edge_attr = f32c(edge_attr, "edge_attr")
        if edge_attr.shape != (ne, encoder.in_dim) or encoder.precision != BF16_N16:
            raise CgnnError("edge_stream: edge_attr must be [E, encoder fan-in] and the encoder packed 'bf16_n16'")
        latent = encoder.out_dim
        if e_out is None:
            e_out = TiledRows(ne, latent, src.device)
    else:
        if not isinstance(e_in, TiledRows):
            raise CgnnError("edge_stream: edge latents must be TiledRows")
        latent = e_in.width
        if e_out is None:
            e_out = e_in.empty_like()
    for t, name in ((ps_all, "ps_all"), (pd_all, "pd_all")):
        require_device(t, name)
        if t.dtype != torch.bfloat16 or not t.is_contiguous() or t.dim() != 3 or t.shape[0] != rounds:
            raise CgnnError(f"edge_stream: {name} must be a contiguous bfloat16 [rounds, N, H] table")
    if any(m.precision != BF16_N16 for m in mlps):
        raise CgnnError("edge_stream: the edge models must be packed 'bf16_n16'")
    if dst.numel() != ne or e_out.n != ne or e_out.width != latent or (e_in is not None and e_in.n != ne):
        raise CgnnError("edge_stream: src/dst/e_out do not match the edge latents")
    arr = (Mlp * rounds)(*[m.struct() for m in mlps])
    enc = encoder.struct() if encoder is not None else None
    with _timed("edge_stream", src.device):
        check(_lib.load().cgnn_edge_stream(arr, rounds, ps_all.data_ptr(), pd_all.data_ptr(),
                                           ps_all.stride(0), src.data_ptr(), dst.data_ptr(), ne,
                                           e_in.buf.data_ptr() if e_in is not None else None, e_out.buf.data_ptr(), latent,
                                           C.byref(enc) if enc is not None else None, ptr(edge_attr),
                                           edge_attr.stride(0) if edge_attr is not None else 0,
                                           stream_ptr(src.device)), "cgnn_edge_stream")
    return e_out


class StreamImage:

    @staticmethod
    def supported(latent: int, hidden: int, nh: int, rounds: int, enc_in: Optional[int] = None) -> bool:
        if hidden != latent or rounds < 1 or (enc_in is not None and enc_in > 16):
            return False
        return _lib.load().cgnn_edge_stream_image_bytes(latent, nh, rounds, 1 if enc_in is not None else 0) > 0

    def __init__(self, mlps: Sequence[PackedMLP], encoder: Optional[PackedMLP] = None, kernel: str = "tile32",
                 folded: bool = False):
        lib = _lib.load()
        if kernel not in ("tile32", "tile32w"):
            raise CgnnError(f"StreamImage: unknown kernel {kernel!r}")
        self.kernel = kernel
        self.folded = bool(folded)
        self.rounds = len(mlps)
        self.latent = mlps[0].out_dim
        self.nh = mlps[0].num_hidden_layers
        self.enc_in = encoder.in_dim if encoder is not None else 0
        if any(m.precision != BF16 for m in mlps) or (encoder is not None and encoder.precision != BF16):
            raise CgnnError("StreamImage: the edge models must be packed 'bf16'")
        nbytes = lib.cgnn_edge_stream_image_bytes(self.latent, self.nh, self.rounds, 1 if encoder is not None else 0)
        if nbytes == 0:
            raise CgnnError(f"StreamImage: latent {self.latent} is not built (hidden == latent in {{32, 64, 128}})")
        dev = mlps[0].layers[0].packed.device
        self.buf = torch.empty(nbytes, dtype=torch.uint8, device=dev)
        arr = (Mlp * self.rounds)(*[m.struct() for m in mlps])
        enc = encoder.struct() if encoder is not None else None
        build = lib.cgnn_edge_stream_image_build_w8 if kernel == "tile32w" else lib.cgnn_edge_stream_image_build
        check(build(arr, self.rounds, C.byref(enc) if enc is not None else None, self.latent, self.buf.data_ptr(), nbytes,
                    stream_ptr(dev)), "cgnn_edge_stream_image_build")
        self._keep = (list(mlps), encoder)


def stream_w8_supported(latent: int, nh: int, fixed_k: int) -> bool:
    return bool(_lib.load().cgnn_edge_stream_w8_supported(latent, nh, int(fixed_k)))


def edge_stream_run(image: StreamImage, ps_all: torch.Tensor, pd_all: torch.Tensor, src: torch.Tensor, dst: torch.Tensor,
                    e_in: Optional[TiledRows], e_out: Optional[TiledRows] = None,
                    edge_attr: Optional[torch.Tensor] = None, kernel: str = "tile32", lag: int = 1,
                    fixed_k: int = 0, folded: Optional[bool] = None) -> TiledRows:
    if kernel not in ("tile32", "tile32w"):
        raise CgnnError(f"edge_stream_run: unknown kernel {kernel!r}")
    if image.kernel != kernel:
        raise CgnnError(f"edge_stream_run: the image was built for {image.kernel!r}, not {kernel!r} (StreamImage(..., kernel=...))")
    src, dst = i32c(src, "src"), i32c(dst, "dst")
    ne, latent = src.numel(), image.latent
    if image.enc_in:
        if edge_attr is None:
            raise CgnnError("edge_stream_run: this image starts with the encoder and needs edge_attr")
        edge_attr = f32c(edge_attr, "edge_attr")
        if edge_attr.shape != (ne, image.enc_in):
            raise CgnnError(f"edge_stream_run: edge_attr must be [E, {image.enc_in}]")
        e_in = None
    elif not isinstance(e_in, TiledRows) or e_in.n != ne or e_in.width != latent:
        raise CgnnError("edge_stream_run: e_in must be the TiledRows edge latents")
    if e_out is None:
        e_out = TiledRows(ne, latent, src.device) if e_in is None else e_in.empty_like()
    pdt = ps_all.dtype
    if pdt == torch.float16 and (kernel != "tile32w" or lag != 0):
        raise CgnnError("edge_stream_run: float16 (CGNN_P_F16_S32) tables are for kernel='tile32w' with lag=0")
    for t, name in ((ps_all, "ps_all"), (pd_all, "pd_all")):
        require_device(t, name)
        if t.dtype != pdt or pdt not in (torch.bfloat16, torch.float16) or not t.is_contiguous() or t.dim() != 3 or \
                t.shape[0] != image.rounds or t.shape[2] != latent:
            raise CgnnError(f"edge_stream_run: {name} must be a contiguous bfloat16 (or, tile32w, float16) "
                            f"[rounds, N, latent] table")
    if dst.numel() != ne or e_out.n != ne or e_out.width != latent:
        raise CgnnError("edge_stream_run: src/dst/e_out do not match the edge latents")
    args = (image.buf.data_ptr(), image.buf.numel(), latent, image.nh, image.rounds, image.enc_in, ps_all.data_ptr(),
            pd_all.data_ptr(), ps_all.stride(0), src.data_ptr(), dst.data_ptr(), ne,
            e_in.buf.data_ptr() if e_in is not None else None, e_out.buf.data_ptr(), ptr(edge_attr),
            edge_attr.stride(0) if edge_attr is not None else 0)
    with _timed("edge_stream", src.device):
        if kernel == "tile32w":
            fold = image.folded if folded is None else bool(folded)
            check(_lib.load().cgnn_edge_stream_run_w8(*args, int(lag), int(fixed_k),
                                                      _lib.P_F16_S32 if pdt == torch.float16 else _lib.P_BF16_S32,
                                                      _lib.STREAM_FOLDED if (fold and pdt == torch.float16) else 0,
                                                      stream_ptr(src.device)), "cgnn_edge_stream_run_w8")
        else:
            check(_lib.load().cgnn_edge_stream_run(*args, stream_ptr(src.device)), "cgnn_edge_stream_run")
    return e_out


class AggregatePlan:

    MIN_NODES = 8192

    def __init__(self, gather: torch.Tensor, num_nodes: int, fixed_k: int):
        gather = i32c(gather, "gather")
        if gather.numel() != num_nodes * fixed_k:
            raise CgnnError("AggregatePlan: gather must hold fixed_k senders per receiver")
        nbytes = _lib.load().cgnn_aggregate_plan_bytes(num_nodes, fixed_k)
        if nbytes == 0:
            raise CgnnError(f"AggregatePlan: fixed_k={fixed_k} cannot be planned")
        self._gather_ref = weakref.ref(gather)
        self.gather_ptr, self.device = gather.data_ptr(), gather.device
        self.num_nodes, self.fixed_k = num_nodes, fixed_k
        self.version = gather._version
        self.blob = torch.empty(nbytes, dtype=torch.uint8, device=gather.device)
        with _timed("aggregate_plan", gather.device):
            check(_lib.load().cgnn_aggregate_plan_build(gather.data_ptr(), num_nodes, fixed_k, self.blob.data_ptr(),
                                                        stream_ptr(gather.device)), "cgnn_aggregate_plan_build")

    @staticmethod
    def supported(num_nodes: int, fixed_k: int, width: int) -> bool:
        return 0 < fixed_k <= 32 and width % 32 == 0 and num_nodes >= AggregatePlan.MIN_NODES

    @staticmethod
    def of(gather: torch.Tensor, num_nodes: int, fixed_k: int, width: int) -> Optional["AggregatePlan"]:
        if not AggregatePlan.supported(num_nodes, fixed_k, width) or gather.dtype != torch.int32 or not gather.is_cuda:
            return None
        plan = getattr(gather, "_cgnn_aggregate_plan", None)
        if plan is None or plan.version != gather._version or plan.num_nodes != num_nodes or plan.fixed_k != fixed_k:
            plan = AggregatePlan(gather, num_nodes, fixed_k)
            gather._cgnn_aggregate_plan = plan
        return plan


def power_bin_ids(mesh: int, k_edges, device) -> torch.Tensor:
    what = "power_bin_ids"
    e = check_power_edges(k_edges, what)
    m = check_mesh(mesh, what)
    device = torch.device(device)
    if device.type != "cuda":
        raise CgnnError(f"{what}: needs a HIP device (got {device}); this engine has no CPU path")
    ids = torch.empty((m, m, m // 2 + 1), dtype=torch.int32, device=device)
    edges_c = (C.c_float * len(e))(*e)
    with _timed(what, ids.device):
        check(_lib.load().cgnn_power_bin_ids(m, edges_c, len(e) - 1, ids.data_ptr(), stream_ptr(ids.device)),
              "cgnn_power_bin_ids")
    return ids


class PowerPlan:

    _last = {}

    def __init__(self, mesh: int, k_edges, device):
        self.edges = tuple(check_power_edges(k_edges, "PowerPlan"))
        self.mesh, self.num_bins = check_mesh(mesh, "PowerPlan"), len(self.edges) - 1
        ids = power_bin_ids(self.mesh, self.edges, device).reshape(-1)
        self.device, self.num_modes = ids.device, ids.numel()
        sorted_ids, perm = torch.sort(ids, stable=True)
        del ids
        self.perm = perm.to(torch.int32)
        del perm
        self.bin_start = torch.searchsorted(
            sorted_ids, torch.arange(self.num_bins + 1, dtype=torch.int32, device=self.device)).to(torch.int32)

    @staticmethod
    def forget() -> None:
        PowerPlan._last.clear()

    @staticmethod
    def of(mesh: int, k_edges, device) -> "PowerPlan":
        device = torch.device(device)
        if device.type == "cuda" and device.index is None:
            device = torch.device("cuda", torch.cuda.current_device())
        key = (int(mesh), tuple(check_power_edges(k_edges, "PowerPlan")))
        plan = PowerPlan._last.get(device)
        if plan is None or (plan.mesh, plan.edges) != key:
            plan = PowerPlan(mesh, k_edges, device)
            PowerPlan._last[device] = plan
        return plan


def aggregate(table, gather: Optional[torch.Tensor], dst: Optional[torch.Tensor], num_nodes: int,
              fixed_k: int = 0, num_edges: Optional[int] = None, out: Optional[torch.Tensor] = None,
              plan: Optional[AggregatePlan] = None) -> torch.Tensor:
    if plan is not None:
        table = f32c(table, "table")
        if gather is None or gather.data_ptr() != plan.gather_ptr or gather.dtype != torch.int32:
            raise CgnnError("aggregate: the plan was built for another sender list")
        if plan.version != gather._version:
            raise CgnnError("aggregate: the sender list changed after the plan was built")
        if fixed_k != plan.fixed_k or num_nodes != plan.num_nodes or table.shape[1] % 32:
            raise CgnnError("aggregate: the plan does not match this call")
        if out is None:
            out = torch.empty((num_nodes, table.shape[1]), dtype=torch.float32, device=table.device)
        _same_device(table, gather, plan.blob, out)
        with _timed("aggregate", table.device):
            check(_lib.load().cgnn_aggregate_planned_rows(table.data_ptr(), table.shape[0], gather.data_ptr(),
                                                          plan.blob.data_ptr(), num_nodes, fixed_k, table.shape[1],
                                                          out.data_ptr(), stream_ptr(table.device)),
                  "cgnn_aggregate_planned")
        return out
    if isinstance(table, TiledRows):
        tb, layout, width, dev, nrows = table.buf, _lib.TILED32, table.width, table.device, table.n
    else:
        table = f32c(table, "table")
        tb, layout, width, dev, nrows = table, _lib.ROWS, table.shape[1], table.device, table.shape[0]
    if gather is not None:
        gather = i32c(gather, "gather")
    if dst is not None:
        dst = i32c(dst, "dst")
    if num_edges is None:
        num_edges = gather.numel() if gather is not None else (dst.numel() if dst is not None else nrows)
    if gather is None and nrows < num_edges:
        raise CgnnError(f"aggregate: a table of {nrows} rows read by edge id for {num_edges} edges")
    if out is None:
        out = torch.empty((num_nodes, width), dtype=torch.float32, device=dev)
    elif tuple(out.shape) != (num_nodes, width) or out.dtype != torch.float32 or not out.is_contiguous():
        raise CgnnError(f"aggregate: out must be contiguous float32 {(num_nodes, width)}")
    _same_device(tb, gather, dst, out)
    with _timed("aggregate", dev):
        check(_lib.load().cgnn_aggregate(tb.data_ptr(), layout, ptr(gather), ptr(dst), num_edges, fixed_k, num_nodes,
                                         width, out.data_ptr(), stream_ptr(dev)), "cgnn_aggregate")
    return out


def node_block(mlp: PackedMLP, w_x: PackedLinear, w_agg: PackedLinear, x: torch.Tensor, agg: torch.Tensor,
               x_out: Optional[torch.Tensor] = None, residual: bool = True, next_projection=None) -> torch.Tensor:
    x, agg = f32c(x, "x"), f32c(agg, "agg")
    n, latent = x.shape
    if x_out is None:
        x_out = torch.empty_like(x)
    sx, sa = w_x.struct(), w_agg.struct()
    if next_projection is not None:
        ws, wd, ps, pd, p_format = next_projection
        s1, s2 = ws.struct(), wd.struct()
        pdt = p_format_dtype(p_format)
        for t in (ps, pd):
            require_device(t, "projection table")
            if t.dtype != pdt or not t.is_contiguous() or t.shape != (n, ws.out_dim):
                raise CgnnError("node_block: projection tables have the wrong dtype/shape")
        proj = (C.byref(s1), C.byref(s2), ws.precision, ps.data_ptr(), pd.data_ptr(), p_format)
    else:
        proj = (None, None, 0, None, None, 0)
    _same_device(x, agg, x_out)
    with _timed("node_block", x.device):
        check(_lib.load().cgnn_node_block(C.byref(mlp.struct()), C.byref(sx), C.byref(sa), x.data_ptr(), agg.data_ptr(),
                                          n, x_out.data_ptr(), 1 if residual else 0, latent, *proj,
                                          stream_ptr(x.device)), "cgnn_node_block")
    return x_out


KNN_GRIDS = ("uniform", "adaptive")


def check_knn_grid(grid: str, who: str) -> str:
    if grid not in KNN_GRIDS:
        raise ValueError(f"{who}: k-NN grid {grid!r}; known: {KNN_GRIDS}")
    return grid


def check_min_image(flag: bool, who: str) -> bool:
    if not isinstance(flag, bool):
        raise TypeError(f"{who}: min_image_edge_attr must be a bool, got {flag!r}")
    return flag


def knn_periodic(pos: torch.Tensor, box_size: float, k: int, query_ids: Optional[torch.Tensor] = None,
                 want_edge_attr: bool = True, want_order: bool = False, *, min_image_edge_attr: bool = False,
                 grid: str = "uniform"):
    check_knn_grid(grid, "knn_periodic")
    check_min_image(min_image_edge_attr, "knn_periodic")
    lib = _lib.load()
    if grid == "adaptive":
        ws_fn, knn_fn, order_fn = (lib.cgnn_knn_adaptive_workspace_bytes, lib.cgnn_knn_periodic_adaptive,
                                   lib.cgnn_knn_adaptive_sorted_order)
        if min_image_edge_attr:
            knn_fn = lib.cgnn_knn_periodic_adaptive_mode
    else:
        ws_fn, knn_fn, order_fn = lib.cgnn_knn_workspace_bytes, lib.cgnn_knn_periodic, lib.cgnn_knn_sorted_order
        if min_image_edge_attr:
            knn_fn = lib.cgnn_knn_periodic_mode
    mode = (_lib.KNN_EDGE_ATTR_IMAGE,) if min_image_edge_attr else ()
    pos = f32c(pos, "pos")
    if pos.dim() != 2 or pos.shape[1] != 3:
        raise CgnnError(f"knn_periodic: pos must be [n, 3], got {tuple(pos.shape)}")
    n = pos.shape[0]
    if query_ids is not None:
        query_ids = i32c(query_ids, "query_ids")
        nq = query_ids.numel()
    else:
        nq = n
    ws_bytes = ws_fn(n, k)
    ws = torch.empty(ws_bytes, dtype=torch.uint8, device=pos.device)
    senders = torch.empty(nq * k, dtype=torch.int32, device=pos.device)
    edge_attr = torch.empty((nq * k, 4), dtype=torch.float32, device=pos.device) if want_edge_attr else None
    st = stream_ptr(pos.device)
    with _timed("knn_periodic", pos.device):
        check(knn_fn(pos.data_ptr(), n, float(box_size), k, ptr(query_ids), nq, senders.data_ptr(),
                     ptr(edge_attr), ws.data_ptr(), ws_bytes, st, *mode), knn_fn.__name__)
    order = None
    if want_order:
        order = torch.empty(n, dtype=torch.int32, device=pos.device)
        check(order_fn(ws.data_ptr(), n, order.data_ptr(), st), order_fn.__name__)
    return senders, edge_attr, order


def check_batch_offsets(offsets, who: str) -> List[int]:
    if torch.is_tensor(offsets):
        if offsets.is_cuda:
            raise CgnnError(f"{who}: offsets are host values (a list or a CPU tensor), got a tensor on {offsets.device}")
        offsets = offsets.tolist()
    offsets = [int(o) for o in offsets]
    if len(offsets) < 2 or offsets[0] != 0 or any(b <= a for a, b in zip(offsets, offsets[1:])):
        raise ValueError(f"{who}: offsets must hold B + 1 >= 2 strictly increasing values starting at 0, got {offsets}")
    return offsets


def knn_periodic_batched(pos: torch.Tensor, offsets, box_size: float, k: int, want_edge_attr: bool = True,
                         want_order: bool = False, *, min_image_edge_attr: bool = False, grid: str = "uniform"):
    what = "knn_periodic_batched"
    check_knn_grid(grid, what)
    check_min_image(min_image_edge_attr, what)
    offsets = check_batch_offsets(offsets, what)
    pos = f32c(pos, "pos")
    if pos.dim() != 2 or pos.shape[1] != 3 or pos.shape[0] != offsets[-1]:
        raise CgnnError(f"{what}: pos must be [{offsets[-1]}, 3] (offsets[-1] rows), got {tuple(pos.shape)}")
    n, num_graphs, k = offsets[-1], len(offsets) - 1, int(k)
    if grid == "adaptive":
        parts = [knn_periodic(pos[a:b], box_size, k, None, want_edge_attr, want_order,
                              min_image_edge_attr=min_image_edge_attr, grid="adaptive")
                 for a, b in zip(offsets, offsets[1:])]
        return (torch.cat([p[0] + a for p, a in zip(parts, offsets)]),
                torch.cat([p[1] for p in parts]) if want_edge_attr else None,
                torch.cat([p[2] + a for p, a in zip(parts, offsets)]) if want_order else None)
    lib = _lib.load()
    offs = (C.c_int64 * (num_graphs + 1))(*offsets)
    ws_bytes = lib.cgnn_knn_batched_workspace_bytes(offs, num_graphs, k)
    ws = torch.empty(ws_bytes, dtype=torch.uint8, device=pos.device)
    senders = torch.empty(n * k, dtype=torch.int32, device=pos.device)
    edge_attr = torch.empty((n * k, 4), dtype=torch.float32, device=pos.device) if want_edge_attr else None
    mode = _lib.KNN_EDGE_ATTR_IMAGE if min_image_edge_attr else _lib.KNN_EDGE_ATTR_REFERENCE
    st = stream_ptr(pos.device)
    with _timed(what, pos.device):
        check(lib.cgnn_knn_periodic_batched(pos.data_ptr(), offs, num_graphs, float(box_size), k, senders.data_ptr(),
                                            ptr(edge_attr), ws.data_ptr(), ws_bytes, st, mode),
              "cgnn_knn_periodic_batched")
    order = None
    if want_order:
        order = torch.empty(n, dtype=torch.int32, device=pos.device)
        check(lib.cgnn_knn_batched_sorted_order(ws.data_ptr(), offs, num_graphs, order.data_ptr(), st),
              "cgnn_knn_batched_sorted_order")
    return senders, edge_attr, order


def check_pair_count_edges(edges, box_size: float, who: str) -> List[float]:
    box = torch.tensor(float(box_size), dtype=torch.float32)
    if not (bool(torch.isfinite(box)) and float(box) > 0.0):
        raise ValueError(f"{who}: box_size must be positive and finite, got {box_size!r}")
    e = torch.as_tensor(edges).detach().to(device="cpu", dtype=torch.float32).reshape(-1)
    nb = e.numel() - 1
    if not 1 <= nb <= _lib.PAIR_COUNTS_MAX_BINS:
        raise ValueError(f"{who}: edges must hold nb + 1 radii with 1 <= nb <= {_lib.PAIR_COUNTS_MAX_BINS}, got "
                         f"{e.numel()} values")
    if not bool(torch.isfinite(e).all()) or float(e[0]) < 0.0 or not bool((e[1:] > e[:-1]).all()):
        raise ValueError(f"{who}: edges must be finite, start at 0 or above and ascend strictly (in float32)")
    if not bool(e[-1] <= box * 0.5):
        raise ValueError(f"{who}: the largest radius {float(e[-1])} exceeds half the box, {float(box) * 0.5}")
    return e.tolist()


def _check_in_box(what: str, box_size: float, **positions) -> None:
    for name, p in positions.items():
        if p is not None and not bool(((p >= 0) & (p <= float(box_size))).all()):
            raise ValueError(f"{what}: {name} leaves [0, box_size]")


def _pair_frames(what: str, pos_a, pos_b, box_size: float, check_bounds: bool):
    pos_a = f32c(pos_a, "pos_a")
    batched = pos_a.dim() == 3
    if pos_a.dim() not in (2, 3) or pos_a.shape[-1] != 3 or pos_a.shape[-2] < 1:
        raise CgnnError(f"{what}: pos_a must be [N, 3] or [T, N, 3] with N >= 1, got {tuple(pos_a.shape)}")
    if pos_b is not None:
        pos_b = f32c(pos_b, "pos_b")
        if pos_b.dim() != pos_a.dim() or pos_b.shape[-1] != 3 or pos_b.shape[-2] < 1 or \
                (batched and pos_b.shape[0] != pos_a.shape[0]):
            raise CgnnError(f"{what}: pos_b must be [M, 3] (or [T, M, 3] with pos_a's T) with M >= 1, got "
                            f"{tuple(pos_b.shape)} for pos_a {tuple(pos_a.shape)}")
        _same_device(pos_a, pos_b)
    if check_bounds:
        _check_in_box(what, box_size, pos_a=pos_a, pos_b=pos_b)
    if batched:
        return pos_a, pos_b, True
    return pos_a.unsqueeze(0), None if pos_b is None else pos_b.unsqueeze(0), False


# ... 1690 lines not shown
```

include/cgnn.h:

```cpp
#ifndef CGNN_H_
#define CGNN_H_

#include <stddef.h>
#include <stdint.h>

#ifdef __cplusplus
extern "C" {
#endif

#define CGNN_VERSION 100
#define CGNN_MAX_HIDDEN_LAYERS 6

typedef enum {
    CGNN_OK = 0,
    CGNN_ERR_INVALID_ARG = -1,
    CGNN_ERR_UNSUPPORTED = -2,
    CGNN_ERR_WORKSPACE = -3,
    CGNN_ERR_HIP = -4
} cgnn_status;

typedef enum {
    CGNN_F32 = 0,
    CGNN_BF16 = 1,
    CGNN_BF16_N16 = 2,
    CGNN_F32X3 = 3,
    CGNN_F32X3_N16 = 4,
    CGNN_F16X2_N16 = 5,
    CGNN_F16X2 = 6
} cgnn_precision;

typedef enum { CGNN_P_F32 = 0, CGNN_P_BF16_S32 = 1, CGNN_P_BF16_S16 = 2, CGNN_P_F16_S32 = 3 } cgnn_ptable;

typedef enum { CGNN_ROWS = 0, CGNN_TILED32 = 1 } cgnn_layout;

typedef struct {
    const void* w;
    const float* b;
    int32_t in_dim;
    int32_t out_dim;
} cgnn_linear;

typedef struct {
    int32_t precision;
    int32_t num_hidden_layers;
    cgnn_linear layer[CGNN_MAX_HIDDEN_LAYERS + 1];
    const float* ln_gamma;
    const float* ln_beta;
} cgnn_mlp;

int cgnn_version(void);
const char* cgnn_arch(void);
const char* cgnn_last_error(void);

size_t cgnn_packed_linear_bytes(int32_t out_dim, int32_t ncols, int32_t precision);
int cgnn_pack_linear(const float* w, int32_t out_dim, int32_t ld, int32_t col0, int32_t ncols,
                     int32_t precision, void* packed, void* stream);

int cgnn_mlp_rows(const cgnn_mlp* mlp, const float* x, int64_t n, int32_t ld_x,
                  float* y, int32_t ld_y, int32_t y_layout, void* stream);

int cgnn_mlp_rows_project(const cgnn_mlp* mlp, const float* x, const int32_t* index, int64_t n, int32_t ld_x, float* y,
                          int32_t ld_y, const cgnn_linear* ws, const cgnn_linear* wd, int32_t proj_precision, void* ps,
                          void* pd, int32_t p_format, void* stream);

int64_t cgnn_tiled_rows(int64_t n);
int cgnn_relayout(const float* src, int32_t from, float* dst, int32_t to, int64_t n, int32_t width, void* stream);

int cgnn_project_nodes(const cgnn_linear* ws, const cgnn_linear* wd, int32_t precision,
                       const float* x, int64_t n, void* ps, void* pd, int32_t p_format, void* stream);

int cgnn_edge_block(const cgnn_mlp* mlp, const void* ps, const void* pd,
                    const int32_t* src, const int32_t* dst, int64_t num_edges,
                    const float* e_in, float* e_out, float* e_upd, int32_t residual,
                    int32_t latent, const float* x_gather, float* agg_out, int32_t seg_k, void* stream);

int cgnn_aggregate(const float* table, int32_t table_layout, const int32_t* gather, const int32_t* dst,
                   int64_t num_edges, int32_t fixed_k, int64_t num_nodes, int32_t width,
                   float* out, void* stream);

size_t cgnn_aggregate_plan_bytes(int64_t num_nodes, int32_t fixed_k);
int cgnn_aggregate_plan_build(const int32_t* gather, int64_t num_nodes, int32_t fixed_k, void* plan, void* stream);
int cgnn_aggregate_planned(const float* table, const int32_t* gather, const void* plan, int64_t num_nodes,
                           int32_t fixed_k, int32_t width, float* out, void* stream);
int cgnn_aggregate_planned_rows(const float* table, int64_t table_rows, const int32_t* gather, const void* plan,
                                int64_t num_nodes, int32_t fixed_k, int32_t width, float* out, void* stream);
int32_t cgnn_aggregate_planned_form(int64_t table_rows, int64_t num_nodes, int32_t fixed_k, int32_t width);

int cgnn_node_block(const cgnn_mlp* mlp, const cgnn_linear* w_x, const cgnn_linear* w_agg,
                    const float* x, const float* agg, int64_t n, float* x_out,
                    int32_t residual, int32_t latent,
                    const cgnn_linear* ws_next, const cgnn_linear* wd_next, int32_t proj_precision,
                    void* ps_next, void* pd_next, int32_t p_format, void* stream);

int cgnn_edge_stream(const cgnn_mlp* rounds, int32_t num_rounds, const void* ps_all, const void* pd_all,
                     int64_t round_stride, const int32_t* src, const int32_t* dst, int64_t num_edges,
                     const float* e_in, float* e_out, int32_t latent, const cgnn_mlp* encoder, const float* edge_attr,
                     int32_t ld_attr, void* stream);

size_t cgnn_edge_stream_image_bytes(int32_t latent, int32_t num_hidden_layers, int32_t num_rounds, int32_t with_encoder);
int cgnn_edge_stream_image_build(const cgnn_mlp* rounds, int32_t num_rounds, const cgnn_mlp* encoder, int32_t latent,
                                 void* image, size_t image_bytes, void* stream);
int cgnn_edge_stream_run(const void* image, size_t image_bytes, int32_t latent, int32_t num_hidden_layers,
                         int32_t num_rounds, int32_t enc_in_dim, const void* ps_all, const void* pd_all,
                         int64_t round_stride, const int32_t* src, const int32_t* dst, int64_t num_edges,
                         const float* e_in, float* e_out, const float* edge_attr, int32_t ld_attr, void* stream);

#define CGNN_STREAM_FOLDED 1
int cgnn_edge_stream_w8_supported(int32_t latent, int32_t num_hidden_layers, int32_t fixed_k);
int cgnn_edge_stream_image_build_w8(const cgnn_mlp* rounds, int32_t num_rounds, const cgnn_mlp* encoder, int32_t latent,
                                    void* image, size_t image_bytes, void* stream);
int cgnn_edge_stream_run_w8(const void* image, size_t image_bytes, int32_t latent, int32_t num_hidden_layers,
                            int32_t num_rounds, int32_t enc_in_dim, const void* ps_all, const void* pd_all,
                            int64_t round_stride, const int32_t* src, const int32_t* dst, int64_t num_edges,
                            const float* e_in, float* e_out, const float* edge_attr, int32_t ld_attr, int32_t lag,
                            int32_t fixed_k, int32_t p_format, int32_t flags, void* stream);

typedef struct {
    float* h[CGNN_MAX_HIDDEN_LAYERS];
    float* g_a[CGNN_MAX_HIDDEN_LAYERS];
    float* g_o;
    float* zhat;
} cgnn_mlp_bwd_buffers;

int cgnn_mlp_backward(const cgnn_mlp* fwd, const cgnn_linear* fwd_part2, const cgnn_mlp* bwd,
                      const cgnn_linear* bwd_part2, const float* u1, int32_t ld1, const float* u2, int32_t ld2,
                      const float* dy, int32_t ld_dy, int64_t n, const cgnn_mlp_bwd_buffers* buf,
                      float* du1, int32_t ld_du1, float* du2, int32_t ld_du2, void* stream);

int cgnn_edge_mlp_backward(const cgnn_mlp* fwd, const cgnn_mlp* bwd, const void* ps, const void* pd, const int32_t* src,
                           const int32_t* dst, int64_t num_edges, const float* e_in, const float* d_agg,
                           const float* de_in, const cgnn_mlp_bwd_buffers* buf, float* dy, float* de_out,
                           int32_t de_out_layout, void* stream);

int cgnn_linear2_rows(const cgnn_linear* wa, const cgnn_linear* wb, int32_t precision, const float* a, const float* b,
                      int64_t n, const float* add1, const float* add2, float* out, void* stream);

int cgnn_weight_grad(const float* g, int32_t ld_g, int32_t out_dim, const float* a, int32_t ld_a, int32_t in_dim,
                     int64_t n, float* dw, int32_t ld_dw, int32_t col0, float* db, void* stream);

size_t cgnn_weight_grad_workspace_bytes(int64_t n, int32_t out_dim, int32_t in_dim);
int cgnn_weight_grad_ordered(const float* g, int32_t ld_g, int32_t out_dim, const float* a, int32_t ld_a, int32_t in_dim,
                             int64_t n, float* dw, int32_t ld_dw, int32_t col0, float* db, void* workspace,
                             size_t workspace_bytes, void* stream);

size_t cgnn_weight_grad_x3_workspace_bytes(void);
int cgnn_weight_grad_x3(const float* g, int32_t ld_g, const float* a, int32_t ld_a, int64_t n, float* dw, int32_t ld_dw,
                        int32_t col0, float* db, void* workspace, size_t workspace_bytes, void* stream);

int cgnn_col_dot(const float* a, int32_t ld_a, const float* b, int32_t ld_b, int64_t n, int32_t width, float* out,
                 void* stream);
int cgnn_col_dot2(const float* a, int32_t ld_a, const float* b, int32_t ld_b, int64_t n, int32_t width, float* out_ab,
                  float* out_a, void* stream);

size_t cgnn_col_dot_workspace_bytes(int64_t n, int32_t width);
int cgnn_col_dot_ordered(const float* a, int32_t ld_a, const float* b, int32_t ld_b, int64_t n, int32_t width, float* out_ab,
                         float* out_a, void* workspace, size_t workspace_bytes, void* stream);

size_t cgnn_csr_workspace_bytes(int64_t num_rows);
int cgnn_csr_build(const int32_t* key, const int32_t* val, int64_t num_edges, int64_t num_rows, int32_t* row_ptr,
                   int32_t* col, void* workspace, size_t workspace_bytes, void* stream);
int cgnn_aggregate_csr(const float* table, const int32_t* row_ptr, const int32_t* col, int64_t num_rows, int32_t width,
                       float* out, void* stream);
int cgnn_aggregate_csr_add(const float* table, const int32_t* row_ptr, const int32_t* col, int64_t num_rows,
                           int32_t width, const float* add1, const float* add2, float* out, void* stream);

size_t cgnn_knn_workspace_bytes(int64_t n, int32_t k);
int cgnn_knn_periodic(const float* pos, int64_t n, float box_size, int32_t k,
                      const int32_t* query_ids, int64_t nq,
                      int32_t* senders, float* edge_attr,
                      void* workspace, size_t workspace_bytes, void* stream);
int cgnn_knn_sorted_order(const void* workspace, int64_t n, int32_t* perm, void* stream);

#define CGNN_KNN_ADAPTIVE_BYTES_PER_PARTICLE 104
#define CGNN_KNN_ADAPTIVE_BYTES_FIXED 4096
size_t cgnn_knn_adaptive_workspace_bytes(int64_t n, int32_t k);
int cgnn_knn_periodic_adaptive(const float* pos, int64_t n, float box_size, int32_t k,
                               const int32_t* query_ids, int64_t nq,
                               int32_t* senders, float* edge_attr,
                               void* workspace, size_t workspace_bytes, void* stream);
int cgnn_knn_adaptive_sorted_order(const void* workspace, int64_t n, int32_t* perm, void* stream);

#define CGNN_KNN_EDGE_ATTR_REFERENCE 0
#define CGNN_KNN_EDGE_ATTR_IMAGE 1
int cgnn_knn_periodic_mode(const float* pos, int64_t n, float box_size, int32_t k,
                           const int32_t* query_ids, int64_t nq,
                           int32_t* senders, float* edge_attr,
                           void* workspace, size_t workspace_bytes, void* stream, int32_t edge_attr_mode);
int cgnn_knn_periodic_adaptive_mode(const float* pos, int64_t n, float box_size, int32_t k,
                                    const int32_t* query_ids, int64_t nq,
                                    int32_t* senders, float* edge_attr,
                                    void* workspace, size_t workspace_bytes, void* stream, int32_t edge_attr_mode);

#define CGNN_KNN_BATCH_GROUP 64
size_t cgnn_knn_batched_workspace_bytes(const int64_t* offsets, int32_t num_graphs, int32_t k);
int cgnn_knn_periodic_batched(const float* pos, const int64_t* offsets, int32_t num_graphs, float box_size, int32_t k,
                              int32_t* senders, float* edge_attr, void* workspace, size_t workspace_bytes,
                              void* stream, int32_t edge_attr_mode);
int cgnn_knn_batched_sorted_order(const void* workspace, const int64_t* offsets, int32_t num_graphs,
                                  int32_t* perm, void* stream);

size_t cgnn_pair_counts_workspace_bytes(int64_t n_a, int64_t n_b, int32_t num_bins);
int cgnn_pair_counts(const float* pos_a, int64_t n_a, const float* pos_b, int64_t n_b, float box_size,
                     const float* edges, int32_t num_bins, int64_t* counts,
                     void* workspace, size_t workspace_bytes, void* stream);

size_t cgnn_pair_counts_smu_workspace_bytes(int64_t n_a, int64_t n_b, int32_t num_s, int32_t num_mu);
int cgnn_pair_counts_smu(const float* pos_a, int64_t n_a, const float* pos_b, int64_t n_b, float box_size,
                         const float* s_edges, int32_t num_s, const float* mu_edges, int32_t num_mu, int32_t los,
                         int64_t* counts , void* workspace, size_t workspace_bytes, void* stream);

size_t cgnn_pair_velocity_sums_workspace_bytes(int64_t n_a, int64_t n_b, int32_t num_bins);
int cgnn_pair_velocity_sums(const float* pos_a, const int32_t* q_a, int64_t n_a, const float* pos_b, const int32_t* q_b,
                            int64_t n_b, float box_size, const float* edges, int32_t num_bins, int64_t* counts,
                            int64_t* sums , void* workspace, size_t workspace_bytes, void* stream);

size_t cgnn_frame_errors_workspace_bytes(int64_t frames, int64_t n);
int cgnn_frame_errors(const float* pred_pos, const float* true_pos, const float* pred_tmp, const float* true_tmp,
                      int64_t frames, int64_t n, float box_size, double* out,
                      void* workspace, size_t workspace_bytes, void* stream);

int cgnn_mass_assign_weighted(const float* pos, const int32_t* q, int64_t frames, int64_t n, int32_t channels,
                              float box_size, int32_t mesh, int32_t order, int64_t* out, void* stream);
int cgnn_mass_assign_weighted_backward(const float* pos, const int32_t* q, const double* d_field, int64_t frames,
                                       int64_t n, int32_t channels, float box_size, int32_t mesh, int32_t order,
                                       double scale_pos, double scale_val, float* d_pos, float* d_val, void* stream);
int cgnn_mass_assign(const float* pos, int64_t frames, int64_t n, float box_size, int32_t mesh, int32_t order,
                     int64_t* out, void* stream);
int cgnn_mass_assign_backward(const float* pos, const double* d_mesh, int64_t frames, int64_t n, float box_size,
                              int32_t mesh, int32_t order, double scale, float* d_pos, void* stream);
int cgnn_power_bin_ids(int32_t mesh, const float* k_edges, int32_t num_bins, int32_t* ids, void* stream);
size_t cgnn_power_bins_workspace_bytes(int64_t frames, int32_t num_bins);
int cgnn_power_bins(const double* a, const double* b, int64_t frames, int32_t mesh, int32_t order, const int32_t* perm,
                    const int32_t* bin_start, int32_t num_bins, int64_t* modes, double* sums,
                    void* workspace, size_t workspace_bytes, void* stream);

int cgnn_redshift_positions(const float* pos, const float* pos_prev, int64_t frames, int64_t n, float box_size,
                            int32_t los, float shift, float* out, void* stream);
size_t cgnn_power_multipoles_workspace_bytes(int64_t frames, int32_t num_bins);
int cgnn_power_multipoles(const double* a, const double* b, const double* a2, const double* b2, int64_t frames,
                          int32_t mesh, int32_t order, int32_t los, const int32_t* perm, const int32_t* bin_start,
                          int32_t num_bins, int64_t* modes, double* sums, void* workspace, size_t workspace_bytes,
                          void* stream);

size_t cgnn_fof_labels_workspace_bytes(int64_t n);
int cgnn_fof_labels(const float* pos, int64_t n, float box_size, float linking_length, int32_t* labels,
                    void* workspace, size_t workspace_bytes, void* stream);
int cgnn_fof_catalogue(const float* pos, const int32_t* labels, int64_t n, float box_size, int32_t* size, int64_t* disp,
                       const int32_t* size_edges, int32_t num_bins, int64_t* hist, void* stream);

size_t cgnn_halo_match_workspace_bytes(int64_t n);
int cgnn_halo_match(const int32_t* labels_a, const int32_t* size_a, const int32_t* labels_b, const int32_t* size_b,
                    int64_t n, int32_t min_a, int32_t min_b, int32_t* match_ab, int32_t* shared_ab, int32_t* match_ba,
                    int32_t* shared_ba, const int32_t* size_edges, int32_t num_bins, int64_t* summary, void* workspace,
                    size_t workspace_bytes, void* stream);
int cgnn_fof_group_sums(const int32_t* labels, const int32_t* q, int64_t n, int32_t channels, int64_t* sums,
                        void* stream);

size_t cgnn_halo_profiles_workspace_bytes(int64_t n, int64_t num_centres);
int cgnn_halo_profiles(const float* pos, int64_t n, const float* centres, int64_t num_centres, float box_size,
                       const float* edges, int32_t num_bins, const int32_t* q, int32_t channels, int64_t* counts,
                       int64_t* sums, void* workspace, size_t workspace_bytes, void* stream);

int cgnn_window_features(const float* pos_seq, const float* temp_seq, const float* pos_noise, const float* temp_noise,
                         int32_t window, int64_t n, float box_size, float dt, float vel_mean, float vel_std,
                         float temp_mean, float temp_std, float* x, float* recent_pos, void* stream);

int cgnn_window_features_rows(const float* pos_seq, const float* temp_seq, int32_t window, int64_t n_total,
                              const int64_t* rows, int64_t n_rows, float box_size, float dt, float vel_mean,
                              float vel_std, float temp_mean, float temp_std, float* x, float* recent_pos,
                              void* stream);

int cgnn_training_sample(const float* pos_seq, const float* temp_seq, const float* target_pos, const float* target_temp,
                         int32_t window, int64_t n_total, const int64_t* rows, int64_t n_rows, double noise_std,
                         uint64_t seed, uint64_t draw, float box_size, float dt, float vel_mean, float vel_std,
                         float temp_mean, float temp_std, const float* stats, float* x, float* recent_pos, float* y_acc,
                         float* y_temp_rate, float* pos_noise, float* temp_noise, void* stream);

int cgnn_training_sample_backward(const float* d_x, const float* d_recent_pos, const float* d_y_acc,
                                  const float* d_y_temp_rate, int32_t window, int64_t n_total, const int64_t* rows,
                                  int64_t n_rows, int32_t first_frame, float box_size, float dt, float vel_std,
                                  float temp_std, const float* stats, float* d_pos, float* d_temp, void* stream);
int cgnn_rollout_integrate_backward(const float* d_new_pos, const float* d_new_temp, int64_t n_rows, const float* stats,
                                    float dt, float box_size, float* d_acc_pred, float* d_temp_rate_pred, float* d_p1,
                                    float* d_p2, float* d_t1, void* stream);
int cgnn_edge_attr_backward(const float* d_edge_attr, const float* edge_attr, const int32_t* senders, int64_t n,
                            int32_t k, const int32_t* row_ptr, const int32_t* col, float* d_pos, void* stream);
int cgnn_edge_attr_backward_rows(const float* d_edge_attr, const float* edge_attr, const int32_t* senders,
                                 int64_t n_recv, int64_t n_pos, int32_t k, const int32_t* row_ptr, const int32_t* col,
                                 float* d_pos, void* stream);
int cgnn_rows_to_frames(const float* rows_pos, const float* rows_temp, const int64_t* ids, int32_t frames, int64_t n_rows,
                        int64_t n_total, float* frames_pos, float* frames_temp, void* stream);
int cgnn_frame_grad_rows(const float* grad, const int64_t* ids, int64_t n_rows, int64_t n_total, float* d_new_pos,
                         float* d_new_temp, void* stream);

#define CGNN_ROLLOUT_ROW 5
int cgnn_rollout_integrate(const float* pos_prev2, const float* pos_prev1, const float* temp_prev1, int64_t n_total,
                           const float* acc_pred, const float* temp_rate_pred, const int64_t* ids, int64_t n_rows,
                           int64_t n_out, const float* stats, float dt, float box_size, float* out, void* stream);
int cgnn_frame_unpack(const float* rows, int64_t n_rows, int64_t n_total, float* pos, float* temp, void* stream);

size_t cgnn_balanced_planes_workspace_bytes(int64_t n, int32_t px, int32_t py, int32_t pz);
int cgnn_balanced_planes(const float* pos, int64_t n, int32_t px, int32_t py, int32_t pz, float* planes_x,
                         float* planes_y, float* planes_z, int32_t* owner, void* workspace, size_t workspace_bytes,
                         void* stream);
int cgnn_tile_classify(const float* pos, int64_t n, int32_t px, int32_t py, int32_t pz, const float* planes_x,
                       const float* planes_y, const float* planes_z, int32_t rank, const double* lo, const double* hi,
                       double margin, double box_size, int32_t* owner, int64_t* counts, uint8_t* mask, void* stream);

#define CGNN_MIGRATE_BLOCK 256
int cgnn_history_features(const float* hist, int32_t window, int64_t cap, int64_t n_held, int32_t phase,
                          const int32_t* rows, int64_t n_rows, const int32_t* ids, float box_size, float dt,
                          float vel_mean, float vel_std, float temp_mean, float temp_std, float* x, float* recent,
                          void* stream);
int cgnn_rollout_advance(float* hist, int32_t window, int64_t cap, int64_t n_held, int32_t phase, const int32_t* ids,
                         const int32_t* pred_row, const float* acc_pred, const float* temp_rate_pred, int64_t n_pred,
                         const float* stats, float dt, float box_size, int32_t px, int32_t py, int32_t pz,
                         int32_t use_planes, const float* planes_x, const float* planes_y, const float* planes_z,
                         float* record, int32_t* dest, int32_t* block_counts, int32_t* counts, void* stream);
int cgnn_halo_select(const float* recent, int64_t n, int32_t world, int32_t rank, const double* lo, const double* hi,
                     double margin, double box_size, uint64_t* mask, int32_t* block_counts, int32_t* counts,
                     void* stream);
int cgnn_halo_pack(const float* recent, const uint64_t* mask, int64_t n, int32_t world, const int32_t* offsets,
                   int64_t n_out, float* out, void* stream);
int cgnn_migrate_pack(const float* hist, int32_t window, int64_t cap, int64_t n_held, const int32_t* ids,
                      const int32_t* dest, int32_t world, int32_t rank, const int32_t* offsets, float* hist_out,
                      int64_t cap_out, int32_t* ids_out, float* send, int64_t n_send, void* stream);
int cgnn_migrate_unpack(const float* recv, int64_t n_recv, int32_t window, float* hist_out, int64_t cap_out,
                        int64_t first, int32_t* ids_out, void* stream);

int cgnn_segment_colsum(const float* acc, const int32_t* batch, int64_t n, int32_t width,
                        int32_t num_graphs, double* sums, void* stream);

int cgnn_gather_rows(const float* table, const int32_t* idx, int64_t n_idx, int32_t width,
                     float* out, void* stream);
int cgnn_scatter_rows(const float* rows, const int32_t* idx, int64_t n_idx, int32_t width,
                      float* table, void* stream);

int cgnn_halo_return_add(const float* ret, int64_t num_ret, const int32_t* rows, const int32_t* seg_ptr,
                         const int32_t* col, int64_t num_rows, int32_t width, float* table, int64_t table_rows,
                         void* stream);

#ifdef __cplusplus
}
#endif
#endif
```

Measured before the change: 6.290 billion edge-updates/s.

## Keep bias and LayerNorm vectors resident in LDS for the folded w8 edge stream

Adds a resident-vector variant of the w8 edge stream kernel. At kernel start it copies every round's bias, LayerNorm gamma and beta vectors into an LDS table, and shrinks each ring slot to the weight bytes only. This removes the per-step DMA of the vector section and the LNBUF copy between passes. The cost is extra LDS per block and a one-off table load at startup. The variant is used by default for folded runs with 1-2 hidden layers when the table fits, and a TRAVELLING flag opts out.

```diff
diff --git a/cosmology_gnn_simulation_amd/_lib.py b/cosmology_gnn_simulation_amd/_lib.py
--- a/cosmology_gnn_simulation_amd/_lib.py
+++ b/cosmology_gnn_simulation_amd/_lib.py
@@ -14,6 +14,7 @@
 N16_NODE = (F32X3_N16, F16X2_N16)
 P_F32, P_BF16_S32, P_BF16_S16, P_F16_S32 = 0, 1, 2, 3
 STREAM_FOLDED = 1
+STREAM_TRAVELLING = 4
 LDS_WEIGHT_BUDGET = 152 * 1024
 PRECISIONS = {"fp32": F32, "f32": F32, "float32": F32, "bf16": BF16, "bfloat16": BF16, "bf16_n16": BF16_N16,
               "fp32x3": F32X3, "f32x3": F32X3, "fp32x3_n16": F32X3_N16, "fp16x2_n16": F16X2_N16,
@@ -28,7 +29,7 @@
     "cgnn_mlp_backward", "cgnn_weight_grad", "cgnn_weight_grad_x3_workspace_bytes", "cgnn_weight_grad_x3",
     "cgnn_col_dot", "cgnn_col_dot2", "cgnn_col_dot_workspace_bytes", "cgnn_col_dot_ordered", "cgnn_weight_grad_workspace_bytes", "cgnn_weight_grad_ordered", "cgnn_csr_workspace_bytes", "cgnn_csr_build",
     "cgnn_aggregate_csr", "cgnn_aggregate_csr_add", "cgnn_edge_stream", "cgnn_edge_stream_image_bytes", "cgnn_edge_stream_image_build",
-    "cgnn_edge_stream_run", "cgnn_edge_stream_w8_supported", "cgnn_edge_stream_image_build_w8", "cgnn_edge_stream_run_w8", "cgnn_aggregate_plan_bytes", "cgnn_aggregate_plan_build", "cgnn_aggregate_planned", "cgnn_aggregate_planned_rows",
+    "cgnn_edge_stream_run", "cgnn_edge_stream_w8_supported", "cgnn_edge_stream_w8_vectors_resident", "cgnn_edge_stream_image_build_w8", "cgnn_edge_stream_run_w8", "cgnn_aggregate_plan_bytes", "cgnn_aggregate_plan_build", "cgnn_aggregate_planned", "cgnn_aggregate_planned_rows",
     "cgnn_aggregate_planned_form", "cgnn_edge_mlp_backward", "cgnn_linear2_rows", "cgnn_halo_return_add", "cgnn_window_features_rows",
     "cgnn_rollout_integrate", "cgnn_frame_unpack", "cgnn_training_sample",
     "cgnn_balanced_planes_workspace_bytes", "cgnn_balanced_planes", "cgnn_tile_classify",
@@ -127,6 +128,7 @@
     lib.cgnn_edge_stream_image_build.argtypes = [C.POINTER(Mlp), i32, C.POINTER(Mlp), i32, vp, sz, vp]
     lib.cgnn_edge_stream_run.argtypes = [vp, sz, i32, i32, i32, i32, vp, vp, i64, vp, vp, i64, vp, vp, vp, i32, vp]
     lib.cgnn_edge_stream_w8_supported.argtypes = [i32, i32, i32]
+    lib.cgnn_edge_stream_w8_vectors_resident.argtypes = [i32, i32, i32, i32]
     lib.cgnn_edge_stream_image_build_w8.argtypes = [C.POINTER(Mlp), i32, C.POINTER(Mlp), i32, vp, sz, vp]
     lib.cgnn_edge_stream_run_w8.argtypes = [vp, sz, i32, i32, i32, i32, vp, vp, i64, vp, vp, i64, vp, vp, vp, i32, i32, i32, i32, i32, vp]
     lib.cgnn_aggregate.argtypes = [vp, i32, vp, vp, i64, i32, i64, i32, vp, vp]
diff --git a/cosmology_gnn_simulation_amd/csrc/edge_stream32w.hip b/cosmology_gnn_simulation_amd/csrc/edge_stream32w.hip
--- a/cosmology_gnn_simulation_amd/csrc/edge_stream32w.hip
+++ b/cosmology_gnn_simulation_amd/csrc/edge_stream32w.hip
@@ -12,15 +12,16 @@
 #define CGNN_IC(x) std::integral_constant<int, (x)> {}
 #include "w8_dev.hpp"
 
-template <int DT>
+template <int DT, bool RESV = false>
 struct W8Geom {
     typedef S32Geom<DT> G;
     static constexpr int D = G::D, KS = G::KS;
-    static constexpr unsigned STRIDE = G::STRIDE, VEC_OFF = G::VEC_OFF;
-    static constexpr int PIECES = (int)(STRIDE / 1024u);
+    static constexpr unsigned IMG_STRIDE = G::STRIDE, VEC_OFF = G::VEC_OFF;
+    static constexpr unsigned STRIDE = RESV ? G::W_BYTES : G::STRIDE;
+    static constexpr int PIECES = (int)((RESV || w8dev::ABL_RING4 ? G::W_BYTES : G::STRIDE) / 1024u);
     static constexpr int NP = (PIECES + CGNN_W8_WAVES - 1) / CGNN_W8_WAVES;
     static constexpr unsigned LNBUF_OFF = CGNN_W8_SLOTS * STRIDE;
-    static constexpr unsigned LNBUF_BYTES = 2u * D * 4u;
+    static constexpr unsigned LNBUF_BYTES = RESV ? 0u : 2u * D * 4u;
     static constexpr unsigned PDST_OFF = LNBUF_OFF + 2u * LNBUF_BYTES;
     static constexpr unsigned PDST_ROW = 256u + 16u;
     static constexpr unsigned PDST_BYTES = 4u * PDST_ROW;
@@ -28,7 +29,14 @@
     static constexpr unsigned PSST_BYTES = 64u * (unsigned)D / 2u;
     static constexpr unsigned LDS = PSST_OFF + CGNN_W8_WAVES * PSST_BYTES;
     static_assert(LDS <= 160u * 1024u, "LDS budget");
+    static constexpr unsigned TABLE_OFF = LDS, TABLE_ROW = (unsigned)D * 4u;
+    static constexpr unsigned TABLE_MAX = RESV ? 160u * 1024u - LDS : 0u;
 };
+
+static inline int64_t w8_table_rows(int nh, int rounds, bool has_encoder) {
+    const int64_t passes = (int64_t)rounds + (has_encoder ? 1 : 0);
+    return passes * (nh + 1) + passes + (has_encoder ? 2 : 1);
+}
 
 template <class W, int LAG>
 struct RingW {
@@ -36,10 +44,11 @@
     int count;
     int wave, lane;
     int slot;
+    int step;
     int dma_chunk, dma_slot;
     CGNN_W8_STAMP_MEMBER
     __device__ __forceinline__ RingW(const char* img, int cnt, int w, int l)
-        : image(img), count(cnt), wave(w), lane(l), slot(0), dma_chunk(0), dma_slot(0) {}
+        : image(img), count(cnt), wave(w), lane(l), slot(0), step(0), dma_chunk(0), dma_slot(0) {}
     __device__ __forceinline__ unsigned lds0() const { return (unsigned)(uintptr_t)(LdsWeightPtr)(cgnn_smem); }
     __device__ __forceinline__ unsigned base() const { return lds0() + (unsigned)slot * W::STRIDE; }
     __device__ __forceinline__ unsigned base_next() const {
@@ -47,19 +56,26 @@
     }
     __device__ __forceinline__ unsigned vec_addr() const { return base() + W::VEC_OFF; }
     __device__ __forceinline__ unsigned lnbuf(int which) const { return lds0() + W::LNBUF_OFF + (unsigned)which * W::LNBUF_BYTES; }
-    __device__ __forceinline__ void piece(int i) {
+    __device__ __forceinline__ unsigned table_row(int row) const { return lds0() + W::TABLE_OFF + (unsigned)row * W::TABLE_ROW; }
+    __device__ __forceinline__ void fetch(int idx, int chunk, int to) {
         asm volatile("" ::: "memory");
 #if defined(__HIP_DEVICE_COMPILE__)
-        int idx = wave + CGNN_W8_WAVES * i;
-        if (idx >= W::PIECES) idx -= CGNN_W8_WAVES;
         const unsigned off = (unsigned)idx * 1024u;
-        char* dst = cgnn_smem + (unsigned)dma_slot * W::STRIDE + off;
+        char* dst = cgnn_smem + (unsigned)to * W::STRIDE + off;
         const __amdgpu_buffer_rsrc_t rsrc =
-            __builtin_amdgcn_make_buffer_rsrc(const_cast<char*>(image), 0, (int)((unsigned)count * W::STRIDE), 0x00020000);
+            __builtin_amdgcn_make_buffer_rsrc(const_cast<char*>(image), 0, (int)((unsigned)count * W::IMG_STRIDE), 0x00020000);
         __builtin_amdgcn_raw_ptr_buffer_load_lds(rsrc, (LdsVoidPtrG)dst, 16, (unsigned)lane * 16u,
-                                                 (unsigned)dma_chunk * W::STRIDE + off, 0, 0);
+                                                 (unsigned)chunk * W::IMG_STRIDE + off, 0, 0);
+#else
+        (void)idx, (void)chunk, (void)to;
 #endif
         asm volatile("" ::: "memory");
+    }
+    __device__ __forceinline__ void piece(int i) {
+        int idx = wave + CGNN_W8_WAVES * i;
+        if constexpr (W::PIECES % CGNN_W8_WAVES != 0)
+            if (idx >= W::PIECES) idx -= CGNN_W8_WAVES;
+        fetch(idx, dma_chunk, dma_slot);
     }
     __device__ __forceinline__ void dma_done() {
         dma_chunk = dma_chunk + 1 == count ? 0 : dma_chunk + 1;
@@ -69,6 +85,9 @@
         for (int c = 0; c < CGNN_W8_SLOTS - 1 - LAG; ++c) {
             for (int i = 0; i < W::NP; ++i) piece(i);
             dma_done();
+        }
+        if constexpr (w8dev::ABL_RING4) {
+            for (int s = 0; s < CGNN_W8_SLOTS; ++s) fetch(W::PIECES + (wave & 3), count - 1, s);
         }
         CGNN_S32_VMCNT(0);
         __builtin_amdgcn_s_barrier();
@@ -85,7 +104,10 @@
         asm volatile("" ::: "memory");
         CGNN_W8_STAMP(K0 + 2);
     }
-    __device__ __forceinline__ void advance() { slot = slot + 1 == CGNN_W8_SLOTS ? 0 : slot + 1; }
+    __device__ __forceinline__ void advance() {
+        slot = slot + 1 == CGNN_W8_SLOTS ? 0 : slot + 1;
+        step = step + 1 == count ? 0 : step + 1;
+    }
     __device__ __forceinline__ void idle_interval() {
         for (int i = 0; i < W::NP; ++i) piece(i);
         dma_done();
@@ -214,16 +236,16 @@
     return st;
 }
 template <bool RES, bool BETA, bool ZM, int DT, int K0, int K1>
-__device__ __forceinline__ void ln_affine_w(const f32x16 (&acc)[DT], f32x16 (&ev)[DT], bf16x8 (&in)[2 * DT], unsigned lnv, int h,
-                                            LnStats st) {
+__device__ __forceinline__ void ln_affine_w(const f32x16 (&acc)[DT], f32x16 (&ev)[DT], bf16x8 (&in)[2 * DT], unsigned lnv, unsigned lnb,
+                                            int h, LnStats st) {
     if constexpr (K1 > K0) {
-        constexpr int D = 32 * DT;
-        const LdsVecPtr gp = (LdsVecPtr)(uintptr_t)lnv + 4 * h;
+        const LdsVecPtr gp = (LdsVecPtr)(uintptr_t)lnv + 4 * h, bp = (LdsVecPtr)(uintptr_t)lnb + 4 * h;
+        (void)bp;
         f32x4 gm[2][2], bt[2][2];
 #pragma unroll
         for (int gg = 0; gg < 2; ++gg) {
             gm[K0 & 1][gg] = *(LdsVec4Ptr)(gp + 32 * (K0 >> 1) + 8 * (2 * (K0 & 1) + gg));
-            if constexpr (BETA) bt[K0 & 1][gg] = *(LdsVec4Ptr)(gp + D + 32 * (K0 >> 1) + 8 * (2 * (K0 & 1) + gg));
+            if constexpr (BETA) bt[K0 & 1][gg] = *(LdsVec4Ptr)(bp + 32 * (K0 >> 1) + 8 * (2 * (K0 & 1) + gg));
         }
         __builtin_amdgcn_sched_barrier(0);
         static_for_each([&](auto kc) __attribute__((always_inline)) {
@@ -233,7 +255,7 @@
 #pragma unroll
                 for (int gg = 0; gg < 2; ++gg) {
                     gm[nxt][gg] = *(LdsVec4Ptr)(gp + 32 * t1 + 8 * (2 * s1 + gg));
-                    if constexpr (BETA) bt[nxt][gg] = *(LdsVec4Ptr)(gp + D + 32 * t1 + 8 * (2 * s1 + gg));
+                    if constexpr (BETA) bt[nxt][gg] = *(LdsVec4Ptr)(bp + 32 * t1 + 8 * (2 * s1 + gg));
                 }
             }
             if constexpr (w8dev::ABL_LN) {
@@ -317,12 +339,13 @@
     }, std::make_integer_sequence<int, T1 - T0>{});
 }
 
-template <int DT, int NH, bool ENC, int LAG, bool PF16, bool FOLD>
+template <int DT, int NH, bool ENC, int LAG, bool PF16, bool FOLD, bool RESV = false>
 __global__ __launch_bounds__(CGNN_W8_BLOCK, 2) void edge_stream32w_kernel(
     S32Args a, const __bf16* __restrict__ ps_all, const __bf16* __restrict__ pd_all, int64_t round_stride,
     const int32_t* __restrict__ src, const int32_t* __restrict__ dst, int64_t num_edges, const float* e_in, float* e_out,
     const float* __restrict__ attr, int ld_attr, int seg_k) {
-    typedef W8Geom<DT> W;
+    typedef W8Geom<DT, RESV> W;
+    static_assert(!RESV || (LAG == 0 && FOLD), "the resident form is built for folded images at lag 0");
     static_assert(DT == 4, "the sender-row staging is laid out for latent 128 (four lanes per 64-byte half line)");
     constexpr int D = W::D, KS = W::KS, NP = W::NP;
     const int lane = threadIdx.x & 63, r = lane & 31, h = lane >> 5;
@@ -338,6 +361,28 @@
     if (iters == 0) return;
     RingW<W, LAG> ring(a.image, steps_per_tile, wave, lane);
     CGNN_W8_STAMP_BEGIN(ring)
+    const int passes = L + (ENC ? 1 : 0);
+    (void)passes;
+    if constexpr (RESV) {
+        const int rows = steps_per_tile + passes + (ENC ? 2 : 1);
+        for (int i = threadIdx.x; i < rows * D; i += CGNN_W8_BLOCK) {
+            const int row = i / D, j = i % D;
+            int chunk = row, vec = 0;
+            if (row >= steps_per_tile + passes) {
+                chunk = (ENC && row == steps_per_tile + passes) ? NH : steps_per_tile - 1;
+                vec = 2;
+            } else if (row >= steps_per_tile) {
+                chunk = (row - steps_per_tile + 1) * (NH + 1) - 1;
+                vec = 1;
+            } else if (ENC && row == NH) {
+                chunk = 0;
+                vec = 1;
+            }
+            const float v = *reinterpret_cast<const float*>(a.image + (size_t)chunk * W::IMG_STRIDE + W::VEC_OFF + (unsigned)(vec * D + j) * 4u);
+            ((__attribute__((address_space(3))) float*)(uintptr_t)ring.table_row(0))[i] = v;
+        }
+        __syncthreads();
+    }
     ring.prime();
     if (lagging) ring.idle_interval();
     const bf16x8 sel0 = p32_selector(lane, 0), sel1 = p32_selector(lane, 1);
@@ -355,6 +400,18 @@
     bf16x8 inb[2][2 * DT];
     bf16x8 ps[2 * DT], pd[2 * DT];
     int lnpar = 0;
+    int pass = 0;
+    unsigned lng = 0, lnb = 0;
+    (void)lnpar, (void)pass;
+    auto bias_addr = [&]() __attribute__((always_inline)) -> unsigned {
+        if constexpr (RESV) return ring.table_row(ring.step); else return ring.vec_addr();
+    };
+    auto pending_ln = [&]() __attribute__((always_inline)) {
+        if constexpr (!RESV) {
+            lng = w8dev::ABL_RING4 ? ring.lds0() + W::VEC_OFF + (unsigned)D * 4u : ring.lnbuf(lnpar ^ 1);
+            lnb = lng + (unsigned)D * 4u;
+        }
+    };
     LnStats lnst = {0.f, 0.f};
     constexpr int KA = CGNN_W8_LN_EARLY < 2 * DT ? CGNN_W8_LN_EARLY : 2 * DT;
     int64_t tile = tr.first < tr.end ? tr.first : tr.end - 1;
@@ -499,7 +556,8 @@
                     static_for_each([&](auto ic) __attribute__((always_inline)) { stage_ps(CGNN_IC(1), ic, tps); },
                                     std::make_integer_sequence<int, 4>{});
                 }
-                ln_affine_w<PEND == 2, !(FOLD && PEND == 2), FOLD, DT, KA, 2 * DT>(acc, ev, inb[0], ring.lnbuf(lnpar ^ 1), h, lnst);
+                pending_ln();
+                ln_affine_w<PEND == 2, !(FOLD && PEND == 2), FOLD, DT, KA, 2 * DT>(acc, ev, inb[0], lng, lnb, h, lnst);
                 if constexpr (!IS_ENC) {
                     if constexpr (INBLK) read_pd_row(CGNN_IC(0)); else read_pd();
                 }
@@ -509,7 +567,7 @@
             constexpr bool REQ = CARRY && !IS_ENC && CGNN_W8_REQ_EARLY;
             if constexpr (REQ) wblock_request<DT * KS0, 0>(fb, base);
             if constexpr (IS_ENC) {
-                bias_rowsw<DT, 0, DT>(acc, ring.vec_addr() + (unsigned)D * 4u, h);
+                bias_rowsw<DT, 0, DT>(acc, RESV ? ring.table_row(NH) : ring.vec_addr() + (unsigned)D * 4u, h);
             } else if constexpr (PEND != 0) {
                 if constexpr (INBLK) {
                     addp_rows<DT, 0, 1>(acc, ps, pd);
@@ -548,12 +606,12 @@
                 if constexpr (t >= 0 && w == (KS0 > 4 ? CGNN_W8_PK0 : (KS0 > 2 ? 1 : KS0 - 1))) packw_slice<true, DT, (t < 0 ? 0 : t), 0>(inb[1], acc);
                 if constexpr (t >= 0 && w == (KS0 > 4 ? CGNN_W8_PK1 : KS0 - 1)) {
                     packw_slice<true, DT, (t < 0 ? 0 : t), 1>(inb[1], acc);
-                    bias_rowsw<DT, (t < 0 ? 0 : t), (t < 0 ? 0 : t) + 1>(acc, ring.vec_addr(), h);
+                    bias_rowsw<DT, (t < 0 ? 0 : t), (t < 0 ? 0 : t) + 1>(acc, bias_addr(), h);
                 }
             }));
             packw_slice<true, DT, DT - 1, 0>(inb[1], acc);
             packw_slice<true, DT, DT - 1, 1>(inb[1], acc);
-            bias_rowsw<DT, DT - 1, DT>(acc, ring.vec_addr(), h);
+            bias_rowsw<DT, DT - 1, DT>(acc, bias_addr(), h);
             ring.dma_done();
             ring.template interval_end<0, 11>();
             ring.advance();
@@ -568,12 +626,12 @@
                 if constexpr (t >= 0 && w == (KS > 4 ? CGNN_W8_PK0 : (KS > 2 ? 1 : KS - 1))) packw_slice<true, DT, (t < 0 ? 0 : t), 0>(inb[(l + 1) & 1], acc);
                 if constexpr (t >= 0 && w == (KS > 4 ? CGNN_W8_PK1 : KS - 1)) {
                     packw_slice<true, DT, (t < 0 ? 0 : t), 1>(inb[(l + 1) & 1], acc);
-                    bias_rowsw<DT, (t < 0 ? 0 : t), (t < 0 ? 0 : t) + 1>(acc, ring.vec_addr(), h);
+                    bias_rowsw<DT, (t < 0 ? 0 : t), (t < 0 ? 0 : t) + 1>(acc, bias_addr(), h);
                 }
             }));
             packw_slice<true, DT, DT - 1, 0>(inb[(l + 1) & 1], acc);
             packw_slice<true, DT, DT - 1, 1>(inb[(l + 1) & 1], acc);
-            bias_rowsw<DT, DT - 1, DT>(acc, ring.vec_addr(), h);
+            bias_rowsw<DT, DT - 1, DT>(acc, bias_addr(), h);
             ring.dma_done();
             ring.template interval_end<0, 15>();
             ring.advance();
@@ -597,16 +655,24 @@
             ln_sums_add<FOLD, DT, DT - 1, 0>(sums, acc);
             ln_sums_add<FOLD, DT, DT - 1, 1>(sums, acc);
             lnst = ln_stats_finish<FOLD, DT>(sums);
-            ln_affine_w<RES, !(FOLD && RES && WITH_P), FOLD, DT, 0, KA>(acc, ev, inb[0], ring.vec_addr() + (unsigned)D * 4u, h, lnst);
-            if (wave < CGNN_W8_WAVES / 2) {
-                const int idx = wave * 64 + lane;
-                if (idx < 2 * D) {
-                    const LdsVecPtr sp = (LdsVecPtr)(uintptr_t)(ring.vec_addr() + (unsigned)D * 4u);
-                    const float v = sp[idx];
-                    ((__attribute__((address_space(3))) float*)(uintptr_t)ring.lnbuf(lnpar))[idx] = v;
-                }
+            if constexpr (RESV) {
+                lng = ring.table_row(steps_per_tile + pass);
+                lnb = ring.table_row(steps_per_tile + passes + (ENC && !IS_ENC ? 1 : 0));
+                pass = pass + 1 == passes ? 0 : pass + 1;
+                ln_affine_w<RES, !(FOLD && RES && WITH_P), FOLD, DT, 0, KA>(acc, ev, inb[0], lng, lnb, h, lnst);
+            } else {
+                ln_affine_w<RES, !(FOLD && RES && WITH_P), FOLD, DT, 0, KA>(acc, ev, inb[0], ring.vec_addr() + (unsigned)D * 4u,
+                                                                             ring.vec_addr() + (unsigned)D * 8u, h, lnst);
+                if (!w8dev::ABL_RING4 && wave < CGNN_W8_WAVES / 2) {
+                    const int idx = wave * 64 + lane;
+                    if (idx < 2 * D) {
+                        const LdsVecPtr sp = (LdsVecPtr)(uintptr_t)(ring.vec_addr() + (unsigned)D * 4u);
+                        const float v = sp[idx];
+                        ((__attribute__((address_space(3))) float*)(uintptr_t)ring.lnbuf(lnpar))[idx] = v;
+                    }
+                }
+                lnpar ^= 1;
             }
-            lnpar ^= 1;
             ring.dma_done();
             ring.template interval_end<(WITH_P && (!CARRY || CGNN_W8_PIECE_SLOT == 0) ? 5 : 0), 3>();
             ring.advance();
@@ -635,7 +701,8 @@
             hidden_steps(ROUND_PASS);
         }
         step_last(ROUND_PASS, std::false_type{}, std::true_type{}, ps_all, pd_all);
-        ln_affine_w<true, true, FOLD, DT, KA, 2 * DT>(acc, ev, inb[0], ring.lnbuf(lnpar ^ 1), h, lnst);
+        pending_ln();
+        if (!RESV || valid) ln_affine_w<true, true, FOLD, DT, KA, 2 * DT>(acc, ev, inb[0], lng, lnb, h, lnst);
 
         if (valid) {
             float* const tb = e_out + tile * (32 * D);
@@ -659,20 +726,25 @@
     __builtin_amdgcn_s_barrier();
 }
 
-template <int DT, int NH, int LAG, bool PF16, bool FOLD>
+template <int DT, int NH, int LAG, bool PF16, bool FOLD, bool RESV = false>
 static int launch_w8(const S32Args& a, const __bf16* ps, const __bf16* pd, int64_t round_stride, const int32_t* src,
                      const int32_t* dst, int64_t num_edges, const float* e_in, float* e_out, const float* attr, int ld_attr,
                      int seg_k, hipStream_t st) {
-    typedef W8Geom<DT> W;
+    typedef W8Geom<DT, RESV> W;
     const bool enc = a.enc_in_dim > 0;
-    auto kern = enc ? edge_stream32w_kernel<DT, NH, true, LAG, PF16, FOLD> : edge_stream32w_kernel<DT, NH, false, LAG, PF16, FOLD>;
-    if (W::LDS > 48 * 1024) {
-        int rc = ensure_dynamic_lds(reinterpret_cast<const void*>(kern), W::LDS, "hipFuncSetAttribute(edge_stream32w)");
+    auto kern = enc ? edge_stream32w_kernel<DT, NH, true, LAG, PF16, FOLD, RESV> : edge_stream32w_kernel<DT, NH, false, LAG, PF16, FOLD, RESV>;
+    const size_t lds = W::LDS + (RESV ? (size_t)w8_table_rows(NH, a.rounds, enc) * W::TABLE_ROW : 0);
+    if (lds > W::LDS + W::TABLE_MAX) {
+        set_error("cgnn_edge_stream_run_w8: the vector table of %d rounds does not fit in LDS", a.rounds);
+        return CGNN_ERR_INVALID_ARG;
+    }
+    if (lds > 48 * 1024) {
+        int rc = ensure_dynamic_lds(reinterpret_cast<const void*>(kern), W::LDS + W::TABLE_MAX, "hipFuncSetAttribute(edge_stream32w)");
         if (rc != CGNN_OK) return rc;
     }
     const int64_t tiles = (num_edges + 31) / 32;
     const int grid = grid_for_tiles(tiles, 1, CGNN_W8_WAVES);
-    kern<<<grid, CGNN_W8_BLOCK, W::LDS, st>>>(a, ps, pd, round_stride, src, dst, num_edges, e_in, e_out, attr, ld_attr, seg_k);
+    kern<<<grid, CGNN_W8_BLOCK, lds, st>>>(a, ps, pd, round_stride, src, dst, num_edges, e_in, e_out, attr, ld_attr, seg_k);
     CGNN_W8_STAMP_REPORT(st, num_edges, grid, a.rounds + (enc ? 1 : 0), LAG)
     return check_hip(hipGetLastError(), "cgnn_edge_stream_run_w8 launch");
 }
@@ -704,6 +776,13 @@
     return (latent == 128 && num_hidden_layers >= 1 && num_hidden_layers <= 3 && k_ok) ? 1 : 0;
 }
 
+extern "C" int cgnn_edge_stream_w8_vectors_resident(int32_t latent, int32_t num_hidden_layers, int32_t num_rounds,
+                                                    int32_t has_encoder) {
+    typedef W8Geom<4, true> W;
+    if (latent != 128 || num_hidden_layers < 1 || num_hidden_layers > 2 || num_rounds < 1) return 0;
+    return w8_table_rows(num_hidden_layers, num_rounds, has_encoder != 0) * (int64_t)W::TABLE_ROW <= (int64_t)W::TABLE_MAX ? 1 : 0;
+}
+
 extern "C" int cgnn_edge_stream_run_w8(const void* image, size_t image_bytes, int32_t latent, int32_t num_hidden_layers,
                                        int32_t num_rounds, int32_t enc_in_dim, const void* ps_all, const void* pd_all,
                                        int64_t round_stride, const int32_t* src, const int32_t* dst, int64_t num_edges,
@@ -719,8 +798,9 @@
                   p_format);
         return CGNN_ERR_INVALID_ARG;
     }
-    if ((flags & ~CGNN_STREAM_FOLDED) != 0 || ((flags & CGNN_STREAM_FOLDED) && p_format != CGNN_P_F16_S32)) {
-        set_error("cgnn_edge_stream_run_w8: flags = %d (known: CGNN_STREAM_FOLDED, with CGNN_P_F16_S32 tables only)", flags);
+    if ((flags & ~(CGNN_STREAM_FOLDED | CGNN_STREAM_TRAVELLING)) != 0 || ((flags & CGNN_STREAM_FOLDED) && p_format != CGNN_P_F16_S32)) {
+        set_error("cgnn_edge_stream_run_w8: flags = %d (known: CGNN_STREAM_FOLDED, with CGNN_P_F16_S32 tables only, and "
+                  "CGNN_STREAM_TRAVELLING)", flags);
         return CGNN_ERR_INVALID_ARG;
     }
     if (p_format == CGNN_P_F16_S32 && lag != 0) {
@@ -755,6 +835,13 @@
     return launch_w8<4, NHx, LAGx, PFx, FOLDx>(a, (const __bf16*)ps_all, (const __bf16*)pd_all, round_stride, src, dst, num_edges, \
                                                e_in, e_out, edge_attr, ld_attr, fixed_k, st)
     if (flags & CGNN_STREAM_FOLDED) {
+        if (!(flags & CGNN_STREAM_TRAVELLING) &&
+            cgnn_edge_stream_w8_vectors_resident(latent, num_hidden_layers, num_rounds, enc_in_dim > 0 ? 1 : 0)) {
+            if (num_hidden_layers == 1) return launch_w8<4, 1, 0, true, true, true>(a, (const __bf16*)ps_all, (const __bf16*)pd_all, round_stride, src, dst,
+                                                                                    num_edges, e_in, e_out, edge_attr, ld_attr, fixed_k, st);
+            return launch_w8<4, 2, 0, true, true, true>(a, (const __bf16*)ps_all, (const __bf16*)pd_all, round_stride, src, dst, num_edges, e_in,
+                                                        e_out, edge_attr, ld_attr, fixed_k, st);
+        }
         switch (num_hidden_layers) {
             case 1: CGNN_W8_GO(1, 0, true, true);
             case 2: CGNN_W8_GO(2, 0, true, true);
diff --git a/cosmology_gnn_simulation_amd/csrc/w8_dev.hpp b/cosmology_gnn_simulation_amd/csrc/w8_dev.hpp
--- a/cosmology_gnn_simulation_amd/csrc/w8_dev.hpp
+++ b/cosmology_gnn_simulation_amd/csrc/w8_dev.hpp
@@ -49,6 +49,11 @@
 constexpr bool ABL_BIAS = true;
 #else
 constexpr bool ABL_BIAS = false;
+#endif
+#ifdef CGNN_W8_ABL_RING4
+constexpr bool ABL_RING4 = true;
+#else
+constexpr bool ABL_RING4 = false;
 #endif
 #ifdef CGNN_W8_SLEEP
 constexpr int SLEEP = CGNN_W8_SLEEP;
diff --git a/cosmology_gnn_simulation_amd/ops.py b/cosmology_gnn_simulation_amd/ops.py
--- a/cosmology_gnn_simulation_amd/ops.py
+++ b/cosmology_gnn_simulation_amd/ops.py
@@ -384,10 +384,14 @@
     return bool(_lib.load().cgnn_edge_stream_w8_supported(latent, nh, int(fixed_k)))
 
 
+def stream_w8_vectors_resident(latent: int, nh: int, rounds: int, has_encoder: bool) -> bool:
+    return bool(_lib.load().cgnn_edge_stream_w8_vectors_resident(latent, nh, rounds, 1 if has_encoder else 0))
+
+
 def edge_stream_run(image: StreamImage, ps_all: torch.Tensor, pd_all: torch.Tensor, src: torch.Tensor, dst: torch.Tensor,
                     e_in: Optional[TiledRows], e_out: Optional[TiledRows] = None,
                     edge_attr: Optional[torch.Tensor] = None, kernel: str = "tile32", lag: int = 1,
-                    fixed_k: int = 0, folded: Optional[bool] = None) -> TiledRows:
+                    fixed_k: int = 0, folded: Optional[bool] = None, travelling: bool = False) -> TiledRows:
     if kernel not in ("tile32", "tile32w"):
         raise CgnnError(f"edge_stream_run: unknown kernel {kernel!r}")
     if image.kernel != kernel:
@@ -425,7 +429,8 @@
             fold = image.folded if folded is None else bool(folded)
             check(_lib.load().cgnn_edge_stream_run_w8(*args, int(lag), int(fixed_k),
                                                       _lib.P_F16_S32 if pdt == torch.float16 else _lib.P_BF16_S32,
-                                                      _lib.STREAM_FOLDED if (fold and pdt == torch.float16) else 0,
+                                                      (_lib.STREAM_FOLDED if (fold and pdt == torch.float16) else 0)
+                                                      | (_lib.STREAM_TRAVELLING if travelling else 0),
                                                       stream_ptr(src.device)), "cgnn_edge_stream_run_w8")
         else:
             check(_lib.load().cgnn_edge_stream_run(*args, stream_ptr(src.device)), "cgnn_edge_stream_run")
diff --git a/include/cgnn.h b/include/cgnn.h
--- a/include/cgnn.h
+++ b/include/cgnn.h
@@ -106,7 +106,9 @@
                          const float* e_in, float* e_out, const float* edge_attr, int32_t ld_attr, void* stream);
 
 #define CGNN_STREAM_FOLDED 1
+#define CGNN_STREAM_TRAVELLING 4
 int cgnn_edge_stream_w8_supported(int32_t latent, int32_t num_hidden_layers, int32_t fixed_k);
+int cgnn_edge_stream_w8_vectors_resident(int32_t latent, int32_t num_hidden_layers, int32_t num_rounds, int32_t has_encoder);
 int cgnn_edge_stream_image_build_w8(const cgnn_mlp* rounds, int32_t num_rounds, const cgnn_mlp* encoder, int32_t latent,
                                     void* image, size_t image_bytes, void* stream);
 int cgnn_edge_stream_run_w8(const void* image, size_t image_bytes, int32_t latent, int32_t num_hidden_layers,
```

Measured after the change: 6.366 billion edge-updates/s (median of 6 runs). +1.2%, better.
